# felixendres/rgbdslam_v2

Measured on AMD Instinct MI355X. Metric: frame-pairs matched+RANSAC/sec, 640x480 ORB-1000, higher is better.
Workload: dtype fp4 MFMA, exact (match) + f32/f64 (RANSAC); 1 GPU; configs[1]: synthetic 640x480 RGB-D, ORB 1000 kp, 20 candidate pairs/frame, 200 frames; max_matches=300, parallelism=pair-sharded x1, graph_capture=True

## Files before the change

rgbdslam_v2_amd/csrc/api_batches.hip:

```cpp
#include "rgbdfe_host.h"

namespace rgbdfe_host {


int fail(rgbdfe_ctx* ctx, int code, const std::string& msg) {
  if (ctx) {
    std::lock_guard<std::mutex> g(ctx->err_mu);
    ctx->last_error = msg;
  }
  return code;
}


void fill_ransac_const(rgbdfe_ctx* ctx) {
  const rgbdfe_params& p = ctx->cfg.params;
  RansacConst& rc = ctx->rc;
  rc.max_matches = p.max_matches;
  rc.min_matches = p.min_matches;
  rc.ransac_iterations = p.ransac_iterations;
  rc.max_dist_m = (float)(double)p.max_dist_for_inliers;
  rc.sq_max_dist = (double)(rc.max_dist_m * rc.max_dist_m);
  rc.depth_cov = p.depth_cov;
  const double cam_angle_x = 58.0 / 180.0 * M_PI;
  const double cam_angle_y = 45.0 / 180.0 * M_PI;
  const double cam_resol_x = 640;
  const double cam_resol_y = 480;
  const double sx = 3 * tan(cam_angle_x / cam_resol_x);
  const double sy = 3 * tan(cam_angle_y / cam_resol_y);
  rc.raster_cov_x = sx * sx;
  rc.raster_cov_y = sy * sy;
  rc.seed = p.seed;
  rc.g2o_iterations = (int32_t)p.g2o_iterations;
}

int validate_params(rgbdfe_ctx* ctx, const rgbdfe_params& p) {
  if (p.max_matches < 1 || p.max_matches > RGBDFE_MAX_MATCHES)
    return fail(ctx, RGBDFE_ERR_INVALID_ARG, "max_matches must be in [1, RGBDFE_MAX_MATCHES]");
  if (p.min_matches < 0 || p.ransac_iterations < 0)
    return fail(ctx, RGBDFE_ERR_INVALID_ARG, "min_matches / ransac_iterations must be >= 0");
  if (!(p.max_dist_for_inliers > 0.f))
    return fail(ctx, RGBDFE_ERR_INVALID_ARG, "max_dist_for_inliers must be > 0");
  if (p.g2o_iterations > 1000u) return fail(ctx, RGBDFE_ERR_INVALID_ARG, "g2o_iterations must be <= 1000");
  if (p.g2o_iterations > 0u && !(p.depth_cov > 0.0))
    return fail(ctx, RGBDFE_ERR_INVALID_ARG, "the g2o refinement needs depth_cov > 0");
  return RGBDFE_OK;
}

int ensure_scratch(rgbdfe_ctx* ctx, size_t bytes) {
  if (bytes <= ctx->scratch_bytes) return RGBDFE_OK;
  if (ctx->d_scratch) (void)hipFree(ctx->d_scratch);
  ctx->d_scratch = nullptr;
  ctx->scratch_bytes = 0;
  HIP_TRY(ctx, hipMalloc(&ctx->d_scratch, bytes));
  ctx->scratch_bytes = bytes;
  return RGBDFE_OK;
}

hipEvent_t get_event(rgbdfe_ctx* ctx) {
  if (!ctx->event_pool.empty()) {
    hipEvent_t e = ctx->event_pool.back();
    ctx->event_pool.pop_back();
    return e;
  }
  hipEvent_t e = nullptr;
  (void)hipEventCreate(&e);
  return e;
}

void drain_pending(rgbdfe_ctx* ctx) {
  for (auto& ln : ctx->lanes)
    if (ln.stream) (void)hipStreamSynchronize(ln.stream);
  for (auto& p : ctx->pending) {
    auto add = [&](int which, hipEvent_t e0, hipEvent_t e1) {
      float ms = 0.f;
      if (hipEventElapsedTime(&ms, e0, e1) == hipSuccess) {
        ctx->k_ms[which] += ms;
        ctx->k_launches[which]++;
        ctx->k_pairs[which] += p.pairs;
      }
    };
    if (p.sift) {
      add(RGBDFE_KERNEL_SIFT_DOT, p.a, p.b);
      add(RGBDFE_KERNEL_SIFT_FINISH, p.b, p.c);
      add(RGBDFE_KERNEL_RANSAC, p.c, p.d);
      ctx->event_pool.push_back(p.d);
    } else {
      add(RGBDFE_KERNEL_HAMMING, p.a, p.b);
      add(RGBDFE_KERNEL_RANSAC, p.b, p.c);
    }
    ctx->event_pool.push_back(p.a);
    ctx->event_pool.push_back(p.b);
    ctx->event_pool.push_back(p.c);
  }
  ctx->pending.clear();
}

int ensure_ec_pool(rgbdfe_ctx* ctx, rgbdfe_ctx::Lane& lane, size_t regions, hipStream_t stream) {
  if (regions <= lane.ec_regions) return RGBDFE_OK;
  HIP_TRY(ctx, hipStreamSynchronize(stream));
  if (lane.d_ec) (void)hipFree(lane.d_ec);
  lane.d_ec = nullptr;
  lane.ec_regions = 0;
  HIP_TRY(ctx, hipMalloc((void**)&lane.d_ec, regions * select_ransac_ec_region_bytes()));
  lane.ec_regions = regions;
  return RGBDFE_OK;
}
int want_latency_path(rgbdfe_ctx* ctx, rgbdfe_ctx::Lane& lane, int32_t n, hipStream_t stream, bool* use, int* chunk_out,
                      PhasePlan* plan) {
  const size_t need_recs = (size_t)n * (size_t)(ctx->rc.ransac_iterations > 0 ? ctx->rc.ransac_iterations : 0);
  const bool force_phases = ctx->latency_chunk_iters < 0;
  const int chunk_cfg = force_phases ? -ctx->latency_chunk_iters : ctx->latency_chunk_iters;
  int chunk = chunk_cfg > 0 ? chunk_cfg : (n <= 64 ? 4 : (n <= 640 ? 7 : (n <= 1280 ? 14 : 28)));
  const int I_all = ctx->rc.ransac_iterations > 0 ? ctx->rc.ransac_iterations : 0;
  const bool too_many_pairs = (size_t)n > kMaxEcRegions;
  while (!too_many_pairs && chunk < I_all && (size_t)n * (size_t)((I_all + chunk - 1) / chunk) > kMaxEcRegions) ++chunk;
  bool latency = !too_many_pairs && n <= ctx->latency_pairs && ctx->rc.ransac_iterations >= 2 * chunk &&
                 need_recs <= ((size_t)1 << 24);
  *chunk_out = chunk;
  if (latency && need_recs > lane.recs_capacity) {
    HIP_TRY(ctx, hipStreamSynchronize(stream));
    if (lane.d_recs) (void)hipFree(lane.d_recs);
    lane.d_recs = nullptr;
    lane.recs_capacity = 0;
    if (hipMalloc((void**)&lane.d_recs, need_recs * (sizeof(IterRec) + sizeof(IterSum)) +
                                            ransac_split_mask_bytes(need_recs, (size_t)ctx->cfg.max_pairs_per_batch)) == hipSuccess)
      lane.recs_capacity = need_recs;
    else latency = false;
  }
  if (latency && !lane.d_walk &&
      hipMalloc((void**)&lane.d_walk, sizeof(WalkState) * ((size_t)ctx->cfg.max_pairs_per_batch + 1)) != hipSuccess) {
    lane.d_walk = nullptr;
    latency = false;
  }
  const int I = ctx->rc.ransac_iterations;
  if (n <= 256 && !force_phases) { plan->n_phases = 1; plan->ends[0] = I; }
  else {
    const int cand[4] = {14, ((I * 7 / 20) / 7) * 7, ((I * 14 / 20) / 7) * 7, I};
    int k = 0, last = 0;
    for (int c : cand) { const int e = c > I ? I : c; if (e > last) { plan->ends[k++] = e; last = e; } }
    if (k == 0) plan->ends[k++] = I;
    plan->n_phases = k;
  }
  *use = latency;
  return ensure_ec_pool(ctx, lane, ((size_t)n + 7) / 8 * 8 + 8, stream);
}

bool hamming_on_mfma(const rgbdfe_ctx* ctx) { return ctx->hamming_mode != 0 && (uint32_t)ctx->cfg.max_keypoints <= 32768u; }

HammingGeometry hamming_geometry(const rgbdfe_ctx* ctx, uint32_t n, uint32_t max_nq, uint32_t max_nt) {
  const uint32_t cap = (uint32_t)ctx->cfg.max_pairs_per_batch;
  if (!hamming_on_mfma(ctx)) {
    HammingGeometry g = hamming_nn_geometry(n, max_nq, max_nt, cap);
    g.shape = 0;
    return g;
  }
  const int pipe_wide = ctx->hamming_mode == 4 ? 1 : ctx->hamming_mode == 3 ? ctx->hamming_wide : 0;
  return hamming_mfma_geometry(n, max_nq, max_nt, cap, pipe_wide, ctx->hamming_mode == 3 ? ctx->hamming_shape : 32);
}

uint32_t launch_hamming(rgbdfe_ctx* ctx, const PairWork* d_work, uint32_t* d_keys, uint32_t n, HammingGeometry geom,
                        hipStream_t stream) {
  const uint32_t mk = (uint32_t)ctx->cfg.max_keypoints;
  if (n > 0 && geom.qblocks > 0) { ctx->hamming_wide_last = (int)geom.wide; ctx->hamming_shape_last = (int)geom.shape; }
  if (hamming_on_mfma(ctx))
    return launch_hamming_mfma(ctx->d_desc4, d_work, d_keys, mk, n, geom, ctx->hamming_mode, stream);
  return launch_hamming_nn(ctx->d_desc, d_work, d_keys, mk, n, geom, stream);
}

uint32_t launch_hamming(rgbdfe_ctx* ctx, const PairWork* d_work, uint32_t* d_keys, uint32_t n, uint32_t max_nq,
                        uint32_t max_nt, hipStream_t stream) {
  return launch_hamming(ctx, d_work, d_keys, n, hamming_geometry(ctx, n, max_nq, max_nt), stream);
}

bool capture_stream_ready(rgbdfe_ctx* ctx) {
  if (ctx->capture_stream) return true;
  if (hipStreamCreateWithFlags(&ctx->capture_stream, hipStreamNonBlocking) != hipSuccess) { (void)hipGetLastError(); ctx->capture_stream = nullptr; }
  return ctx->capture_stream != nullptr;
}

int enqueue_pairs(rgbdfe_ctx* ctx, const int32_t* qids, const int32_t* tids, int32_t n, rgbdfe_match_result* d_out, hipEvent_t wait_for, int64_t* ticket_out, int* lane_out, int matcher, float* d_out_dist, double flann_ratio) {


  const bool sift = matcher != 0;
  if (n > ctx->cfg.max_pairs_per_batch)
    return fail(ctx, RGBDFE_ERR_CAPACITY, "n_pairs exceeds max_pairs_per_batch");
  const int64_t ticket = ctx->next_ticket;
  rgbdfe_ctx::Slot& slot = ctx->ring[ticket % rgbdfe_ctx::kRing];
  const int li = (int)(ticket % rgbdfe_ctx::kLanes);
  rgbdfe_ctx::Lane& lane = ctx->lanes[li];
  hipStream_t stream = lane.stream;
  if (slot.pending) {
    HIP_TRY(ctx, hipEventSynchronize(slot.done));
    slot.pending = false;
  }
  uint32_t max_nq = 0, max_nt = 0, sift_kinds = 0;
  for (int32_t i = 0; i < n; ++i) {
    auto q = ctx->nodes.find(qids[i]);
    auto t = ctx->nodes.find(tids[i]);
    if (q == ctx->nodes.end() || t == ctx->nodes.end())
      return fail(ctx, RGBDFE_ERR_UNKNOWN_NODE, "pair references a node that is not resident");
    if (q->second.kind != (uint32_t)matcher || t->second.kind != (uint32_t)matcher)
      return fail(ctx, RGBDFE_ERR_INVALID_ARG, "node descriptor kind does not fit this matcher");
    PairWork& w = slot.h_work[i];
    w.q_slot = q->second.slot;
    w.t_slot = t->second.slot;
    w.nq = q->second.n;
    w.nt = t->second.n;
    w.uid = pair_uid(qids[i], tids[i]);
    w.qid = qids[i];
    w.tid = tids[i];
    w.pad = matcher == 1 ? sift_fast_keys(ctx, q->second, t->second) : 0u;
    sift_kinds |= w.pad ? 1u : 2u;
    if (ctx->rc.g2o_iterations > 0 && !(q->second.flags & t->second.flags & kNodeHasKeypoints))
      return fail(ctx, RGBDFE_ERR_INVALID_ARG,
                  "g2o_iterations > 0: a node of the batch has no keypoints (rgbdfe_upload_node_keypoints after every upload of it)");
    if (w.nq > max_nq) max_nq = w.nq;
    if (w.nt > max_nt) max_nt = w.nt;
  }
  if (ctx->rc.g2o_iterations > 0 && !ctx->d_kp2d)
    return fail(ctx, RGBDFE_ERR_INVALID_ARG, "g2o_iterations > 0 needs the nodes' keypoints (rgbdfe_upload_node_keypoints)");
  int32_t piece = n;
  if (n > 0 && ctx->latency_pairs != 0) {
    const size_t I = (size_t)(ctx->rc.ransac_iterations > 0 ? ctx->rc.ransac_iterations : 1);
    size_t fit = (((size_t)1 << 24) / I) < kMaxEcRegions ? (((size_t)1 << 24) / I) : kMaxEcRegions;
    if (fit > 65535) fit = 65535;
    if (fit < 1) fit = 1;
    if ((size_t)n > fit && (size_t)n <= (size_t)ctx->latency_pairs) piece = (int32_t)fit;
  }
  if (sift && piece > 65535) return fail(ctx, RGBDFE_ERR_CAPACITY, "a one-wave SIFT batch holds at most 65535 pairs");
  bool latency = false;
  int chunk = 7;
  PhasePlan pp{};
  if (n > 0) {
    int rcl = want_latency_path(ctx, lane, piece, stream, &latency, &chunk, &pp);
    if (rcl != RGBDFE_OK) return rcl;
  }
  if (wait_for) HIP_TRY(ctx, hipStreamWaitEvent(stream, wait_for, 0));
  if (ctx->nodes_ready) HIP_TRY(ctx, hipStreamWaitEvent(stream, ctx->nodes_ready, 0));
  hipError_t launch_err = hipSuccess;
  if (n > 0) {
    if (!d_out) d_out = lane.d_results;
    const bool graphable = ctx->use_graphs && !sift && !ctx->profiling && piece >= n && ctx->rc.g2o_iterations == 0;
    const HammingGeometry geom = sift ? HammingGeometry{0, 1, 0}
                                      : hamming_geometry(ctx, (uint32_t)(piece < n ? piece : n), max_nq, max_nt);
    if (!sift && geom.qblocks > 0) { ctx->hamming_wide_last = (int)geom.wide; ctx->hamming_shape_last = (int)geom.shape; }
    rgbdfe_ctx::GraphEntry* ge = nullptr;
    bool capturing = false;
    if (graphable) {
      rgbdfe_ctx::GraphKey key;
      memset(&key, 0, sizeof(key));
      key.n = n; key.qblocks = geom.qblocks; key.tsplit = geom.tsplit; key.slot = (int32_t)(ticket % rgbdfe_ctx::kRing);
      key.latency = latency ? 1 : 0; key.chunk = chunk; key.hamming_mode = ctx->hamming_mode | (int32_t)(geom.wide << 8) | (int32_t)(geom.shape << 16); key.n_phases = pp.n_phases;
      for (int i = 0; i < 4; ++i) key.ends[i] = i < pp.n_phases ? pp.ends[i] : 0;
      memcpy(&key.rc, &ctx->rc, sizeof(RansacConst));
      key.d_out = d_out; key.d_recs = lane.d_recs; key.d_ec = lane.d_ec; key.d_walk = lane.d_walk; key.d_keys = lane.d_keys;
      size_t gi = 0;
      for (; gi < ctx->graphs.size(); ++gi)
        if (memcmp(&ctx->graphs[gi].key, &key, sizeof(key)) == 0) { ge = &ctx->graphs[gi]; break; }
      if (ge) {
        ge->used = ++ctx->graph_clock;
        const hipError_t le = hipGraphLaunch(ge->exec, stream);
        if (le == hipSuccess) {
          ctx->graph_launches++;
          ctx->graph_miss_run = 0;
        } else {
          (void)hipGetLastError();
          (void)hipGraphExecDestroy(ge->exec); (void)hipGraphDestroy(ge->graph);
          ctx->graphs.erase(ctx->graphs.begin() + (long)gi);
          ctx->graph_launch_failures++;
          ge = nullptr;
        }
      } else {
        ctx->graph_misses++;
        const bool try_capture = ctx->graph_miss_run < rgbdfe_ctx::kGraphMissRun ||
                                 ctx->graph_miss_run % rgbdfe_ctx::kGraphRetry == 0;
        ctx->graph_miss_run++;
        if (try_capture && capture_stream_ready(ctx) &&
            hipStreamBeginCapture(ctx->capture_stream, hipStreamCaptureModeRelaxed) == hipSuccess) {
          capturing = true;
          if (ctx->graphs.size() >= 48) {
            size_t lru = 0;
            for (size_t i = 1; i < ctx->graphs.size(); ++i) if (ctx->graphs[i].used < ctx->graphs[lru].used) lru = i;
            (void)hipGraphExecDestroy(ctx->graphs[lru].exec); (void)hipGraphDestroy(ctx->graphs[lru].graph);
            ctx->graphs.erase(ctx->graphs.begin() + (long)lru);
          }
          ctx->graphs.push_back(rgbdfe_ctx::GraphEntry{key, nullptr, nullptr, ++ctx->graph_clock});
        } else {
          (void)hipGetLastError();
          ctx->graph_plain_batches++;
        }
      }
    }
    rgbdfe_ctx::Pending pend{};
    pend.sift = sift;
    for (int attempt = 0; attempt < 2; ++attempt) {
      hipStream_t const ls = capturing ? ctx->capture_stream : stream;
      if (!ge) {
        const hipError_t me = hipMemcpyAsync(slot.d_work, slot.h_work, sizeof(PairWork) * (size_t)n, hipMemcpyHostToDevice, ls);
        if (me != hipSuccess && launch_err == hipSuccess) launch_err = me;
      }
      if (ctx->profiling) {
        pend.a = get_event(ctx);
        pend.b = get_event(ctx);
        pend.c = get_event(ctx);
        if (sift) pend.d = get_event(ctx);
        pend.pairs = n;
        (void)hipEventRecord(pend.a, ls);
      }
      const uint32_t mk = (uint32_t)ctx->cfg.max_keypoints;
      for (int32_t off = 0; off < n && !ge; off += piece) {
        const int32_t m = (n - off) < piece ? (n - off) : piece;
        const bool first = off == 0, last = off + m >= n;
        if (!first) {
          int rcl = want_latency_path(ctx, lane, m, ls, &latency, &chunk, &pp);
          if (rcl != RGBDFE_OK) { launch_err = hipErrorOutOfMemory; break; }
        }
        const PairWork* d_work = slot.d_work + off;
        rgbdfe_match_result* d_res = d_out + off;
        if (!sift) {
          const uint32_t planes = launch_hamming(ctx, d_work, lane.d_keys, (uint32_t)m, first ? geom : hamming_geometry(ctx, (uint32_t)m, max_nq, max_nt), ls);
          if (ctx->profiling && first) (void)hipEventRecord(pend.b, ls);
          if (latency)
            launch_select_ransac_latency(ctx->d_xyz, d_work, lane.d_keys, planes, d_res, mk, (uint32_t)m, ctx->rc,
                                         lane.d_prep, lane.d_recs, lane.d_walk, lane.d_ec, chunk, pp.ends, pp.n_phases, ls);
          else
            launch_select_ransac(ctx->d_xyz, d_work, lane.d_keys, planes, d_res, mk, (uint32_t)m, ctx->rc, lane.d_prep,
                                 lane.d_ec, ls);
          if (ctx->rc.g2o_iterations > 0)
            launch_g2o_refine(d_work, d_res, (uint32_t)m, ctx->rc, lane.d_prep, ctx->d_kp2d, mk, lane.d_ec, ls);
          if (ctx->profiling && last) (void)hipEventRecord(pend.c, ls);
        } else {
          float* d_dist = (d_out_dist ? d_out_dist : lane.d_all_dist) + (size_t)off * RGBDFE_MAX_MATCHES;
          if (matcher == 2) {
            launch_l2_knn2(ctx->d_sift_f32, d_work, mk, (uint32_t)m, max_nq, lane.d_row_part, ls);
            if (ctx->profiling && first) (void)hipEventRecord(pend.b, ls);
            launch_l2_ratio(d_work, mk, (uint32_t)m, lane.d_row_part, lane.d_col_part, flann_ratio, lane.d_sm_q,
                            lane.d_sm_t, lane.d_sm_d, lane.d_sm_n, ls);
          } else {
            launch_sift_dot(ctx->d_sift_bf16, d_work, mk, (uint32_t)m, max_nq, max_nt, sift_kinds, lane.d_row_part,
                            lane.d_col_part, lane.d_col_blocks, ls);
            if (ctx->profiling && first) (void)hipEventRecord(pend.b, ls);
            launch_sift_finish(ctx->d_sift_f32, d_work, mk, (uint32_t)m, lane.d_row_part, lane.d_col_part, lane.d_col_blocks,
                               lane.d_sm_q, lane.d_sm_t, lane.d_sm_d, lane.d_sm_n, ls);
          }
          if (ctx->profiling && first) (void)hipEventRecord(pend.c, ls);
          if (latency)
            launch_select_ransac_sift_latency(ctx->d_xyz, d_work, lane.d_sm_q, lane.d_sm_t, lane.d_sm_d, lane.d_sm_n,
                                              d_dist, d_res, mk, (uint32_t)m, ctx->rc,
                                              lane.d_prep, lane.d_recs, lane.d_walk, lane.d_ec, chunk, pp.ends, pp.n_phases, ls);
          else
            launch_select_ransac_sift(ctx->d_xyz, d_work, lane.d_sm_q, lane.d_sm_t, lane.d_sm_d,
                                      lane.d_sm_n, d_dist, d_res, mk,
                                      (uint32_t)m, ctx->rc, lane.d_prep, lane.d_ec, ls);
          if (ctx->rc.g2o_iterations > 0)
            launch_g2o_refine(d_work, d_res, (uint32_t)m, ctx->rc, lane.d_prep, ctx->d_kp2d, mk, lane.d_ec, ls);
          if (ctx->profiling && last) (void)hipEventRecord(pend.d, ls);
        }
      }
      if (capturing) {
        rgbdfe_ctx::GraphEntry& e = ctx->graphs.back();
        hipError_t ce = hipStreamEndCapture(ctx->capture_stream, &e.graph);
        if (ce == hipSuccess) ce = hipGraphInstantiate(&e.exec, e.graph, nullptr, nullptr, 0);
        if (ce == hipSuccess && launch_err == hipSuccess) {
          ctx->graph_captures++;
          ce = hipGraphLaunch(e.exec, stream);
          ctx->graph_launches++;
          if (ce != hipSuccess) launch_err = ce;
        } else {
          if (e.exec) (void)hipGraphExecDestroy(e.exec);
          if (e.graph) (void)hipGraphDestroy(e.graph);
          ctx->graphs.pop_back();
          (void)hipGetLastError();
          capturing = false;
          launch_err = hipSuccess;
          ctx->graph_capture_failures++;
          continue;
        }
      }
      break;
    }
    if (launch_err == hipSuccess) launch_err = hipGetLastError();
    if (ctx->profiling) {
      if (launch_err == hipSuccess) ctx->pending.push_back(pend);
      else {
        ctx->event_pool.push_back(pend.a); ctx->event_pool.push_back(pend.b); ctx->event_pool.push_back(pend.c);
        if (sift) ctx->event_pool.push_back(pend.d);
      }
    }
  }
  ctx->next_ticket++;
  slot.ticket = ticket;
  slot.failed = launch_err != hipSuccess;
  HIP_TRY(ctx, hipEventRecord(slot.done, stream));
  slot.pending = true;
  if (launch_err != hipSuccess)
    return fail(ctx, RGBDFE_ERR_HIP, std::string("kernel launch: ") + hipGetErrorString(launch_err));
  if (ticket_out) *ticket_out = ticket;
  if (lane_out) *lane_out = li;
  return RGBDFE_OK;
}

int wait_ticket(rgbdfe_ctx* ctx, int64_t ticket, hipStream_t stream) {
  if (ticket <= 0 || ticket >= ctx->next_ticket) return fail(ctx, RGBDFE_ERR_INVALID_ARG, "unknown ticket");
  rgbdfe_ctx::Slot& slot = ctx->ring[ticket % rgbdfe_ctx::kRing];
  if (slot.ticket == ticket && slot.failed) return fail(ctx, RGBDFE_ERR_HIP, "the batch with this ticket failed to launch");
  if (slot.ticket != ticket || !slot.pending) return RGBDFE_OK;
  if (stream) {
    HIP_TRY(ctx, hipStreamWaitEvent(stream, slot.done, 0));
  } else {
    HIP_TRY(ctx, hipEventSynchronize(slot.done));
    slot.pending = false;
  }
  return RGBDFE_OK;
}


}
```

rgbdslam_v2_amd/csrc/ransac_device.h:

```cpp
#pragma once
#include <float.h>
#include <stddef.h>

#include <type_traits>

#include "rgbdfe_internal.h"
#include "tfc_device.h"

namespace rgbdfe {

constexpr int kWave = 64;
constexpr int kRounds = RGBDFE_MAX_MATCHES / kWave;

constexpr int kSlots = 7;
constexpr int kFitUnroll = 4;
constexpr int kOrdStride = RGBDFE_MAX_MATCHES + 2 * kFitUnroll + 4;
static_assert(kOrdStride % 4 == 0 && (kOrdStride / 4) % 2 == 1, "list rows: word aligned, odd word count");
static_assert(RGBDFE_MAX_MATCHES <= 512, "list entries keep the low 8 bits of a match index + one threshold");

struct FitBuf {
  uint8_t ord[kSlots][kOrdStride];
};

__device__ __forceinline__ uint32_t mix32(uint32_t x) {
// ... 136 lines not shown
  return ((uint64_t)hi << 32) | lo;
}

__device__ __forceinline__ int fit_compact(int s, const uint64_t* mask, const uint64_t* w_nonzero, FitBuf& fit,
                                           int& n_below_256, int lane) {
  uint32_t base = 0;
  n_below_256 = 0;
#pragma unroll
  for (int r = 0; r < kRounds; ++r) {
    const uint64_t pm = mask[r] & w_nonzero[r];
    if (__builtin_amdgcn_inverse_ballot_w64(pm)) fit.ord[s][base + lane_rank(pm)] = (uint8_t)(r * kWave + lane);
    base += (uint32_t)__popcll(pm);
    if (r == 256 / kWave - 1) n_below_256 = (int)base;
  }
  if (lane < 2 * kFitUnroll) fit.ord[s][base + lane] = 0;
  return (int)base;
}

__device__ __forceinline__ void pin(float& v) { asm volatile("" : "+v"(v)); }

template <bool FAST_DIV>
__device__ __forceinline__ void fit_recurrence(int n_mine, int k256_mine, int n_min, int n_max, const FitBuf& fit,
                                               const float* __restrict__ M, float& C, float& m1, float& m2, int lane) {
  constexpr int U = kFitUnroll;
  const int sl = min(lane / 9, kSlots - 1);
  const int l9 = lane % 9;
  const int ci = l9 / 3, cj = l9 % 3;
  const uint8_t* __restrict__ ord = fit.ord[sl];
  auto rec_off = [&](int k) {
    const uint32_t hi = (k >= k256_mine) ? 256u * kRecBytes : 0u;
    return (uint32_t)ord[k] * kRecBytes + hi;
  };
  const char* __restrict__ recs = reinterpret_cast<const char*>(M);
  const char* __restrict__ recP = recs + cj * 4;
  const char* __restrict__ recQ = recs + 12 + ci * 4;
  float W = 0.0f;
  C = 0.0f; m1 = 0.0f; m2 = 0.0f;
  uint32_t off[U];
  float wv[U], fv[U], tv[U];
#pragma unroll
  for (int u = 0; u < U; ++u) off[u] = rec_off(u);
#pragma unroll
  for (int u = 0; u < U; ++u) {
    wv[u] = *reinterpret_cast<const float*>(recs + off[u] + 24);
    fv[u] = *reinterpret_cast<const float*>(recP + off[u]);
    tv[u] = *reinterpret_cast<const float*>(recQ + off[u]);
  }
#pragma unroll
  for (int u = 0; u < U; ++u) off[u] = rec_off(U + u);
  auto trip = [&](int k0, auto with_select) {
    float wc[U], fc[U], tc[U];
#pragma unroll
    for (int u = 0; u < U; ++u) { wc[u] = wv[u]; fc[u] = fv[u]; tc[u] = tv[u]; }
#pragma unroll
    for (int u = 0; u < U; ++u) {
      wv[u] = *reinterpret_cast<const float*>(recs + off[u] + 24);
      fv[u] = *reinterpret_cast<const float*>(recP + off[u]);
      tv[u] = *reinterpret_cast<const float*>(recQ + off[u]);
    }
#pragma unroll
    for (int u = 0; u < U; ++u) off[u] = rec_off(k0 + 2 * U + u);
    float al[U], om[U];
#pragma unroll
    for (int u = 0; u < U; ++u) {
      W = W + wc[u];
      if (FAST_DIV) {
        float r = __builtin_amdgcn_rcpf(W);
        const float e = __builtin_fmaf(-W, r, 1.0f);
        r = __builtin_fmaf(e, r, r);
        float q = wc[u] * r;
        float res = __builtin_fmaf(-W, q, wc[u]);
        q = __builtin_fmaf(res, r, q);
        res = __builtin_fmaf(-W, q, wc[u]);
        al[u] = __builtin_fmaf(res, r, q);
      } else {
        al[u] = wc[u] / W;
      }
      om[u] = 1.0f - al[u];
    }
#pragma unroll
    for (int u = 0; u < U; ++u) {
      const bool act = (k0 + u) < n_mine;
      const float d1 = fc[u] - m1;
      const float d2 = tc[u] - m2;
      const float outer = d2 * d1;
      const float scaled = al[u] * outer;
      const float sum = C + scaled;
      float Cn = om[u] * sum;
      float m1n = m1 + al[u] * d1;
      float m2n = m2 + al[u] * d2;
      if (decltype(with_select)::value) {
        pin(Cn); pin(m1n); pin(m2n);
        C = act ? Cn : C;
        m1 = act ? m1n : m1;
        m2 = act ? m2n : m2;
      } else {
        C = Cn; m1 = m1n; m2 = m2n;
      }
    }
  };
  int k0 = 0;
  for (; k0 + U <= n_min; k0 += U) trip(k0, std::false_type());
  for (; k0 < n_max; k0 += U) trip(k0, std::true_type());
}

__device__ __forceinline__ uint32_t prescreen_may_pass(const float* hypR, const float* hypt, const float* __restrict__ M,
                                                    int n_all, float pmax, const RansacConst& rc) {
  const float u4 = 4.0f * 5.9604645e-8f;
  float es = 0.0f;
#pragma unroll
  for (int i = 0; i < 3; ++i)
    es += u4 * (((fabsf(hypR[3 * i]) + fabsf(hypR[3 * i + 1])) + fabsf(hypR[3 * i + 2]) + 1.0f) * pmax + fabsf(hypt[i]));
  const double smax = rc.raster_cov_x > rc.depth_cov ? rc.raster_cov_x : rc.depth_cov;
  const float S = (float)(2.0 * (smax + smax));
  const float E = 2.0f * ((2.0f * sqrtf(S) * 1.001f) * es + es * es + u4 * S) + 1e-30f;
  const float hi_f = S * 1.000001f + E;
  uint32_t may_pass = 0;
  typedef float v2f __attribute__((ext_vector_type(2)));
  v2f R2[9], t2[3];
#pragma unroll
  for (int i = 0; i < 9; ++i) R2[i] = v2f{hypR[i], hypR[i]};
#pragma unroll
  for (int i = 0; i < 3; ++i) t2[i] = v2f{hypt[i], hypt[i]};
#pragma unroll 1
  for (int m0 = 0; m0 < n_all; m0 += 4) {
    float rec[4][6];
#pragma unroll
    for (int u = 0; u < 4; ++u)
#pragma unroll
      for (int c = 0; c < 6; ++c) rec[u][c] = M[(m0 + u) * kRec + c];
#pragma unroll
    for (int u = 0; u < 4; u += 2) {
      const v2f px = {rec[u][0], rec[u + 1][0]}, py = {rec[u][1], rec[u + 1][1]}, pz = {rec[u][2], rec[u + 1][2]};
      const v2f qx = {rec[u][3], rec[u + 1][3]}, qy = {rec[u][4], rec[u + 1][4]}, qz = {rec[u][5], rec[u + 1][5]};
      const v2f f0 = __builtin_elementwise_fma(R2[0], px, __builtin_elementwise_fma(R2[1], py, __builtin_elementwise_fma(R2[2], pz, t2[0]))) - qx;
      const v2f f1 = __builtin_elementwise_fma(R2[3], px, __builtin_elementwise_fma(R2[4], py, __builtin_elementwise_fma(R2[5], pz, t2[1]))) - qy;
      const v2f f2 = __builtin_elementwise_fma(R2[6], px, __builtin_elementwise_fma(R2[7], py, __builtin_elementwise_fma(R2[8], pz, t2[2]))) - qz;
      const v2f dsq = __builtin_elementwise_fma(f0, f0, __builtin_elementwise_fma(f1, f1, f2 * f2));
      may_pass += !(dsq.x > hi_f) ? 1u : 0u;
      may_pass += !(dsq.y > hi_f) ? 1u : 0u;
    }
  }
  return may_pass;
}

constexpr int kS4Block = 24;
__device__ __forceinline__ void transpose_records(const float* __restrict__ M, float* __restrict__ S4, int tid, int n_threads) {
  for (int v = tid; v < (RGBDFE_MAX_MATCHES / 4) * kS4Block; v += n_threads) {
    const int blk = v / kS4Block, r = v - blk * kS4Block;
    S4[v] = M[(blk * 4 + (r & 3)) * kRec + (r >> 2)];
  }
}
__device__ __forceinline__ uint32_t prescreen_may_pass_s4(const float* hypR, const float* hypt, const float* __restrict__ S4,
                                                       int n_all, float pmax, const RansacConst& rc) {
  const float u4 = 4.0f * 5.9604645e-8f;
  float es = 0.0f;
#pragma unroll
  for (int i = 0; i < 3; ++i)
    es += u4 * (((fabsf(hypR[3 * i]) + fabsf(hypR[3 * i + 1])) + fabsf(hypR[3 * i + 2]) + 1.0f) * pmax + fabsf(hypt[i]));
  const double smax = rc.raster_cov_x > rc.depth_cov ? rc.raster_cov_x : rc.depth_cov;
  const float S = (float)(2.0 * (smax + smax));
  const float E = 2.0f * ((2.0f * sqrtf(S) * 1.001f) * es + es * es + u4 * S) + 1e-30f;
  const float hi_f = S * 1.000001f + E;
  uint32_t may_pass = 0;
  typedef float v2f __attribute__((ext_vector_type(2)));
  typedef float v4f __attribute__((ext_vector_type(4)));
  v2f R2[9], t2[3];
#pragma unroll
  for (int i = 0; i < 9; ++i) R2[i] = v2f{hypR[i], hypR[i]};
#pragma unroll
  for (int i = 0; i < 3; ++i) t2[i] = v2f{hypt[i], hypt[i]};
  const v4f* __restrict__ blocks = reinterpret_cast<const v4f*>(S4);
#pragma unroll 1
  for (int m0 = 0; m0 < n_all; m0 += 4) {
    const v4f* __restrict__ b = blocks + (m0 >> 2) * 6;
    const v4f px = b[0], py = b[1], pz = b[2], qx = b[3], qy = b[4], qz = b[5];
#pragma unroll
    for (int h = 0; h < 2; ++h) {
      const v2f x = h ? px.zw : px.xy, y = h ? py.zw : py.xy, z = h ? pz.zw : pz.xy;
      const v2f f0 = __builtin_elementwise_fma(R2[0], x, __builtin_elementwise_fma(R2[1], y, __builtin_elementwise_fma(R2[2], z, t2[0]))) - (h ? qx.zw : qx.xy);
      const v2f f1 = __builtin_elementwise_fma(R2[3], x, __builtin_elementwise_fma(R2[4], y, __builtin_elementwise_fma(R2[5], z, t2[1]))) - (h ? qy.zw : qy.xy);
      const v2f f2 = __builtin_elementwise_fma(R2[6], x, __builtin_elementwise_fma(R2[7], y, __builtin_elementwise_fma(R2[8], z, t2[2]))) - (h ? qz.zw : qz.xy);
      const v2f dsq = __builtin_elementwise_fma(f0, f0, __builtin_elementwise_fma(f1, f1, f2 * f2));
      may_pass += !(dsq.x > hi_f) ? 1u : 0u;
      may_pass += !(dsq.y > hi_f) ? 1u : 0u;
    }
  }
  return may_pass;
}

struct WalkRegs {
  int it, real_iterations, valid_iterations, best_idx, best_n;
  float rmse;
  bool done;
};
template <bool COHERENT, class Listed>
__device__ __forceinline__ void walk_records(WalkRegs& w, int recorded_end, int I, int n_all, uint32_t thr,
                                             const IterSum* __restrict__ sum_pair, Listed listed, int lane) {
  while (!w.done && w.it < I && w.real_iterations < recorded_end) {
    const int k0 = w.real_iterations;
    const int G = min(kWave, recorded_end - k0);
    int rn_l = 0;
    double rerr_l = 0.0;
    if (lane < G && listed(k0 + lane)) {
      if (COHERENT) {
        const unsigned long long* p = reinterpret_cast<const unsigned long long*>(sum_pair + (k0 + lane));
        const unsigned long long a = __hip_atomic_load(p, __ATOMIC_RELAXED, __HIP_MEMORY_SCOPE_AGENT);
        const unsigned long long b = __hip_atomic_load(p + 1, __ATOMIC_RELAXED, __HIP_MEMORY_SCOPE_AGENT);
        rerr_l = __longlong_as_double((long long)a);
        rn_l = (int)(uint32_t)b;
      } else {
        const IterSum su = sum_pair[k0 + lane];
        rn_l = su.rn;
        rerr_l = su.rerr;
      }
    }
    const uint64_t with_matches = __ballot(lane < G && rn_l > 0);
    for (int g = 0; g < G;) {
      const uint64_t rest = with_matches >> g;
      const int run = rest != 0ull ? (int)__builtin_ctzll(rest) : G - g;
      if (run > 0) {
        const int can = min(run, max(I - w.it, 0));
        w.real_iterations += can;
        w.it += can;
        if (can < run) { w.done = true; break; }
        g += run;
        if (g >= G) break;
      }
      if (!(w.it < I)) { w.done = true; break; }
      w.real_iterations++;
      const int refined_n = __builtin_amdgcn_readlane(rn_l, g);
      const double refined_error = __hiloint2double(__builtin_amdgcn_readlane(__double2hiint(rerr_l), g),
                                                    __builtin_amdgcn_readlane(__double2loint(rerr_l), g));
      w.valid_iterations++;
      if (refined_error <= (double)w.rmse && refined_n >= w.best_n && (uint32_t)refined_n >= thr) {
        w.rmse = (float)refined_error;
        w.best_idx = k0 + g;
        w.best_n = refined_n;
        if ((double)refined_n > (double)n_all * 0.5) w.it += 10;
        if ((double)refined_n > (double)n_all * 0.75) w.it += 10;
        if ((double)refined_n > (double)n_all * 0.8) { w.done = true; break; }
      }
      ++w.it;
      ++g;
    }
  }
}

#ifndef RGBDFE_CLASS2_NUM
#define RGBDFE_CLASS2_NUM 9
#define RGBDFE_CLASS2_DEN 14
#endif
constexpr int kClass2Num = RGBDFE_CLASS2_NUM, kClass2Den = RGBDFE_CLASS2_DEN;

}
```

rgbdslam_v2_amd/csrc/ransac_split.hip:

```cpp
#include <stdio.h>
#include <stdlib.h>

#include <mutex>
#include <vector>

#include "ransac_device.h"

namespace rgbdfe {

namespace {

__device__ __forceinline__ void lsync() {
  __builtin_amdgcn_wave_barrier();
  asm volatile("s_waitcnt lgkmcnt(0)" ::: "memory");
  __builtin_amdgcn_wave_barrier();
}

__device__ __forceinline__ void lds_barrier() {
  asm volatile("s_waitcnt lgkmcnt(0)\n\ts_barrier" ::: "memory");
}

__device__ __forceinline__ int fresh(int v) {
  asm volatile("" : "+v"(v));
  return v;
}

constexpr int kHypThreads = 256;

#ifdef RGBDFE_SPLIT_STATS
__device__ unsigned long long g_split_stats[40];
#define ST_DECL unsigned long long st_c[40] = {0, 0, 0, 0, 0, 0, 0, 0, 0, 0, 0, 0, 0, 0, 0, 0, 0, 0, 0, 0, 0, 0, 0, 0, 0, 0, 0, 0, 0, 0, 0, 0, 0, 0, 0, 0, 0, 0, 0, 0}, st_mx = 0;
#define ST_ADD(I, V) { st_c[I] += (unsigned long long)(V); }
#define ST_MAX(I, V) { st_mx = (unsigned long long)(V) > st_mx ? (unsigned long long)(V) : st_mx; }
#define ST_T0 unsigned long long st_t = __builtin_amdgcn_s_memrealtime();
#define ST_LAP(I) { const unsigned long long st_n = __builtin_amdgcn_s_memrealtime(); st_c[I] += st_n - st_t; st_t = st_n; }
#define ST_OUT { if ((threadIdx.x & 63) == 0) { for (int st_i = 0; st_i < 40; ++st_i) if (st_c[st_i] != 0ull) atomicAdd(&g_split_stats[st_i], st_c[st_i]); \
                 if (st_mx != 0ull) atomicMax(&g_split_stats[7], st_mx); } }
#else
#define ST_DECL
#define ST_ADD(I, V)
#define ST_MAX(I, V)
#define ST_T0
#define ST_LAP(I)
#define ST_OUT
#endif

#ifndef RGBDFE_SPLIT_WAVES
#define RGBDFE_SPLIT_WAVES 8
#endif
constexpr int kStreamWaves = RGBDFE_SPLIT_WAVES;
#ifndef RGBDFE_SPLIT_WGS_PER_CU
#define RGBDFE_SPLIT_WGS_PER_CU (16 / RGBDFE_SPLIT_WAVES)
#endif
constexpr int kWgsPerCu = RGBDFE_SPLIT_WGS_PER_CU;
static_assert(kStreamWaves >= 3 && (kStreamWaves * kWgsPerCu) % 4 == 0, "whole waves per SIMD");
#define RGBDFE_SPLIT_EU_WAVES (RGBDFE_SPLIT_WAVES * RGBDFE_SPLIT_WGS_PER_CU / 4)
constexpr int kWorkers = kStreamWaves - 1;
#ifndef RGBDFE_SPLIT_SERVER_SCORES
#define RGBDFE_SPLIT_SERVER_SCORES (RGBDFE_SPLIT_WAVES >= 8)
#endif
constexpr bool kServerScores = RGBDFE_SPLIT_SERVER_SCORES;
constexpr int kStreamThreads = kStreamWaves * kWave;
#ifndef RGBDFE_SPLIT_WAVE_SLOTS
#define RGBDFE_SPLIT_WAVE_SLOTS 7
#endif
#ifndef RGBDFE_SPLIT_BUFS
#define RGBDFE_SPLIT_BUFS (RGBDFE_SPLIT_WAVES >= 8 ? 4 : 2)
#endif
constexpr int kWaveSlots = RGBDFE_SPLIT_WAVE_SLOTS;
static_assert(kWaveSlots <= kSlots, "the refit phase (fit_compact / fit_recurrence) holds kSlots lists per wave");
constexpr int kGroupSlots = kWorkers * kWaveSlots;
constexpr int kStreamSlots = 2 * kGroupSlots;
static_assert(kGroupSlots <= kWave, "the server looks at a group's slots with one lane each");
static_assert(kStreamSlots <= 2 * kWave, "the server's end-of-work test looks at two slots per lane");
#ifndef RGBDFE_SPLIT_TICKETS_FROM
#define RGBDFE_SPLIT_TICKETS_FROM (24 * (RGBDFE_SPLIT_WAVES - 1) * RGBDFE_SPLIT_WAVE_SLOTS / 49)
#endif
constexpr int kCostDear = 4;
constexpr int kTicketsFrom = RGBDFE_SPLIT_TICKETS_FROM;
#ifndef RGBDFE_SPLIT_PACK_FROM
#define RGBDFE_SPLIT_PACK_FROM 1000
#endif
constexpr int kPackFrom = RGBDFE_SPLIT_PACK_FROM;
constexpr int kBufs = RGBDFE_SPLIT_BUFS;
#ifndef RGBDFE_SPLIT_MAX_SHARE
#define RGBDFE_SPLIT_MAX_SHARE 256
#endif
constexpr int kMaxShare = RGBDFE_SPLIT_MAX_SHARE;
constexpr int kMaskLanes = kMaxShare / kWave + 1;
constexpr int kMVec = RGBDFE_MAX_MATCHES * kRec / 4;
constexpr int kPrepVec = (int)(sizeof(PairPrep) / 16);
static_assert(sizeof(PairPrep) % 16 == 0, "PairPrep goes global -> LDS in 16-byte pieces");

constexpr int kSlotDone = 0, kSlotActive = 1, kSlotRecorded = 2;
struct SlotS {
  union {
    struct { float R[9], t[3]; } x;
    float svd_in[15];
  } u;
  uint64_t cmask[kRounds];
  double rerr;
  double csum;
  int rn;
  int cn;
  int active;
  int round;
  int iter;
  int buf;
  uint32_t pair;
  int n_all;
  uint32_t thr;
  float pmax;
};
struct ScoreB {
  uint16_t cand[RGBDFE_MAX_MATCHES];
  uint32_t mbits[2 * kRounds];
  uint32_t pad[2];
  double err[RGBDFE_MAX_MATCHES + 8];
};
static_assert(offsetof(ScoreB, err) % 16 == 0, "16-byte reads of the error list");
struct alignas(16) WaveLds {
  union {
    ScoreB sc;
    FitBuf fit;
  } u;
};
constexpr int kUnitFree = 0, kUnitLoading = 1, kUnitReady = 2, kUnitDrained = 3;
struct alignas(16) UnitCtx {
  uint64_t mw[kMaskLanes + 1];
  int state;
  int next;
  int done;
  int n_items;
  uint32_t pair;
  int kb, ke;
  uint32_t thr;
  int base;
  int cls;
  int w_it, w_real, w_valid, w_best_idx, w_best_n, w_state;
  float w_rmse;
  int pad[3];
  uint16_t klist[kMaxShare];
};
struct alignas(16) StreamLds {
  PairPrep prep[kBufs];
  WaveLds w[kServerScores ? kStreamWaves : kWorkers];
  SlotS slot[kStreamSlots];
  UnitCtx ctx[kBufs];
  int claim_nall[kWave];
  int claim_cls[kWave];
  uint8_t act_list[2][kWave];
  int n_act[2];
  int task[2];
  int tickets[2];
  uint8_t wlist[2][kWorkers][8];
  int quit[2];
  int sum_rn[2];
  uint16_t ord_cnt[kWave], ord_start[kWave];
#ifdef RGBDFE_SPLIT_STATS
  unsigned int st_w[2][8][2];
#endif
};
static_assert(sizeof(StreamLds) <= 160 * 1024 / kWgsPerCu, "kWgsPerCu workgroups per CU");

__device__ __forceinline__ void score_b(const float* R, const float* tr, const float* __restrict__ M, int n_all,
                                        uint32_t need, const RansacConst& rc, ScoreB& sb, float pmax, uint64_t* mask,
                                        int& n_inl, double& sum, int& n_cand_out) {
  const int lane = threadIdx.x & (kWave - 1);
  double Rd[9], td[3];
#pragma unroll
  for (int i = 0; i < 9; ++i) Rd[i] = (double)R[i];
#pragma unroll
  for (int i = 0; i < 3; ++i) td[i] = (double)tr[i];
  const double rcx = rc.raster_cov_x, rcy = rc.raster_cov_y, dc = rc.depth_cov;
  const double smax = rcx > dc ? rcx : dc;
  const double shortcut = 2.0 * (smax + smax);
  float lo_f, hi_f;
  {
    const float u4 = 4.0f * 5.9604645e-8f;
    float es = 0.0f;
#pragma unroll
    for (int i = 0; i < 3; ++i)
      es += u4 * (((fabsf(R[3 * i]) + fabsf(R[3 * i + 1])) + fabsf(R[3 * i + 2]) + 1.0f) * pmax + fabsf(tr[i]));
    const float S = (float)shortcut;
    const float E = 2.0f * ((2.0f * sqrtf(S) * 1.001f) * es + es * es + u4 * S) + 1e-30f;
    lo_f = S * 0.999999f - E;
    hi_f = S * 1.000001f + E;
  }
  int n_cand = 0;
  float rec[kRounds][6];
#pragma unroll
  for (int r = 0; r < kRounds; ++r) {
    const int m = r * kWave + lane;
#pragma unroll
    for (int c = 0; c < 6; ++c) rec[r][c] = M[m * kRec + c];
  }
  bool pre[kRounds], cand[kRounds];
  bool unsure = false;
#pragma unroll
  for (int r = 0; r < kRounds; ++r) {
    const int m = r * kWave + lane;
    const float pxf = rec[r][0], pyf = rec[r][1], pzf = rec[r][2];
    const float qxf = rec[r][3], qyf = rec[r][4], qzf = rec[r][5];
    pre[r] = (m < n_all) && !(pzf == 0.0f || qzf == 0.0f) && !(__builtin_isnan(pzf) || __builtin_isnan(qzf));
    const float f0 = __builtin_fmaf(R[0], pxf, __builtin_fmaf(R[1], pyf, __builtin_fmaf(R[2], pzf, tr[0]))) - qxf;
    const float f1 = __builtin_fmaf(R[3], pxf, __builtin_fmaf(R[4], pyf, __builtin_fmaf(R[5], pzf, tr[1]))) - qyf;
    const float f2 = __builtin_fmaf(R[6], pxf, __builtin_fmaf(R[7], pyf, __builtin_fmaf(R[8], pzf, tr[2]))) - qzf;
    const float dsq_f = __builtin_fmaf(f0, f0, __builtin_fmaf(f1, f1, f2 * f2));
    const bool sure_in = dsq_f < lo_f, sure_out = dsq_f > hi_f;
    cand[r] = pre[r] && sure_in;
    unsure = unsure || (pre[r] && !(sure_in || sure_out));
  }
  if (__ballot(unsure) != 0ull) {
#pragma unroll
    for (int r = 0; r < kRounds; ++r) {
      const float pxf = rec[r][0], pyf = rec[r][1], pzf = rec[r][2];
      const float qxf = rec[r][3], qyf = rec[r][4], qzf = rec[r][5];
      const double a0 = (double)pxf, a1 = (double)pyf, a2 = (double)pzf;
      const double d0 = (((Rd[0] * a0 + Rd[1] * a1) + Rd[2] * a2) + td[0]) - (double)qxf;
      const double d1 = (((Rd[3] * a0 + Rd[4] * a1) + Rd[5] * a2) + td[1]) - (double)qyf;
      const double d2 = (((Rd[6] * a0 + Rd[7] * a1) + Rd[8] * a2) + td[2]) - (double)qzf;
      const double dsq = (d0 * d0 + d1 * d1) + d2 * d2;
      cand[r] = pre[r] && !(dsq > shortcut) && !__builtin_isnan(d2);
    }
  }
#pragma unroll
  for (int r = 0; r < kRounds; ++r) {
    const uint64_t cm = __ballot(cand[r]);
    if (cand[r]) sb.cand[n_cand + (int)lane_rank(cm)] = (uint16_t)(r * kWave + lane);
    n_cand += __popcll(cm);
  }
  if (lane < 2 * kRounds) sb.mbits[lane] = 0u;
  lsync();
  n_inl = 0;
  sum = 0.0;
#pragma unroll
  for (int r = 0; r < kRounds; ++r) mask[r] = 0ull;
  n_cand_out = n_cand;
  if ((uint32_t)n_cand < need) return;
  for (int k0 = 0; k0 < n_cand; k0 += kWave) {
    const int k = k0 + lane;
    const bool act = k < n_cand;
    const int m = act ? (int)sb.cand[k] : 0;
    const double a0 = (double)M[m * kRec + 0], a1 = (double)M[m * kRec + 1], a2 = (double)M[m * kRec + 2];
    const double b0 = (double)M[m * kRec + 3], b1 = (double)M[m * kRec + 4], b2 = (double)M[m * kRec + 5];
    double d[3];
    d[0] = (((Rd[0] * a0 + Rd[1] * a1) + Rd[2] * a2) + td[0]) - b0;
    d[1] = (((Rd[3] * a0 + Rd[4] * a1) + Rd[5] * a2) + td[1]) - b1;
    d[2] = (((Rd[6] * a0 + Rd[7] * a1) + Rd[8] * a2) + td[2]) - b2;
    double e = DBL_MAX;
    {
      const double c1[3] = {rcx * a2, rcy * a2, dc};
      const double c2[3] = {rcx * b2, rcy * b2, dc};
      double A[9];
#pragma unroll
      for (int i = 0; i < 3; ++i)
#pragma unroll
        for (int kk = 0; kk < 3; ++kk) A[i * 3 + kk] = Rd[kk * 3 + i] * c1[kk];
      const double S00 = ((A[0] * Rd[0] + A[1] * Rd[3]) + A[2] * Rd[6]) + c2[0];
      const double S10 = (A[3] * Rd[0] + A[4] * Rd[3]) + A[5] * Rd[6];
      const double S11 = ((A[3] * Rd[1] + A[4] * Rd[4]) + A[5] * Rd[7]) + c2[1];
      const double S20 = (A[6] * Rd[0] + A[7] * Rd[3]) + A[8] * Rd[6];
      const double S21 = (A[6] * Rd[1] + A[7] * Rd[4]) + A[8] * Rd[7];
      const double S22 = ((A[6] * Rd[2] + A[7] * Rd[5]) + A[8] * Rd[8]) + c2[2];
      bool ok, unsafe;
      double ee = mahal_llt_fast(S00, S10, S11, S20, S21, S22, d, ok, unsafe);
      if (__ballot(act && unsafe) != 0ull)
        ee = mahal_llt_ieee(S00, S10, S11, S20, S21, S22, d, ok);
      if (ok && (ee >= 0.0)) e = ee;
    }
    const bool inl = act && !(e > rc.sq_max_dist) && (e >= 0.0);
    const uint64_t im = __ballot(inl);
    if (inl) {
      sb.err[n_inl + (int)lane_rank(im)] = e;
      atomicOr(&sb.mbits[m >> 5], 1u << (m & 31));
    }
    n_inl += __popcll(im);
  }
  if (lane < 8) sb.err[n_inl + lane] = 0.0;
  lsync();
#pragma unroll
  for (int r = 0; r < kRounds; ++r) {
    const uint32_t lo = __builtin_amdgcn_readfirstlane(sb.mbits[2 * r]);
    const uint32_t hi = __builtin_amdgcn_readfirstlane(sb.mbits[2 * r + 1]);
    mask[r] = ((uint64_t)hi << 32) | lo;
  }
  if (!((uint32_t)n_inl < need || n_inl < 3)) {
    double s = 0.0;
    for (int k = 0; k < n_inl; k += 8) {
      const double2 v0 = *reinterpret_cast<const double2*>(&sb.err[k]);
      const double2 v1 = *reinterpret_cast<const double2*>(&sb.err[k + 2]);
      const double2 v2 = *reinterpret_cast<const double2*>(&sb.err[k + 4]);
      const double2 v3 = *reinterpret_cast<const double2*>(&sb.err[k + 6]);
      s += v0.x; s += v0.y; s += v1.x; s += v1.y;
      s += v2.x; s += v2.y; s += v3.x; s += v3.y;
    }
    sum = s;
  }
  lsync();
}

}

__global__ __launch_bounds__(kHypThreads) void ransac_hyp_kernel(const PairWork* __restrict__ work, uint32_t n_pairs,
                                                                const RansacConst rc, const SplitPlan plan) {
  __shared__ __attribute__((aligned(16))) float M[RGBDFE_MAX_MATCHES * kRec];
  __shared__ __attribute__((aligned(16))) float S4[(RGBDFE_MAX_MATCHES / 4) * kS4Block];
  const uint32_t pair = blockIdx.x;
  if (pair >= n_pairs) return;
  if (pair == 0 && threadIdx.x < sizeof(WalkState) / 4) reinterpret_cast<uint32_t*>(plan.walk + n_pairs)[threadIdx.x] = 0u;
  const PairPrep* __restrict__ pp = plan.prep + pair;
  const int n_all = pp->n_all;
  if (threadIdx.x == 0) {
    WalkState ws;
    ws.state = rc.ransac_iterations;
    ws.it = 0; ws.real_iterations = 0; ws.valid_iterations = 0;
    ws.best_idx = -1; ws.best_n = 0;
    ws.rmse = 1e6f;
    ws.speculate = plan.phased ? 0 : rc.ransac_iterations;
    plan.walk[pair] = ws;
  }
  if (!(n_all > rc.min_matches && n_all >= 4)) return;
  const int tid = threadIdx.x, lane = tid & (kWave - 1);
  {
    const float4* __restrict__ src = reinterpret_cast<const float4*>(pp->M);
    float4* __restrict__ dst = reinterpret_cast<float4*>(M);
    for (int v = tid; v < kMVec; v += kHypThreads) dst[v] = src[v];
  }
  __shared__ int n_viable_sh;
  if (tid == 0) n_viable_sh = 0;
  __syncthreads();
  transpose_records(M, S4, tid, kHypThreads);
  __syncthreads();
  const float pmax = pp->pmax;
  uint32_t thr = (uint32_t)rc.min_matches;
  if ((double)thr > 0.75 * (double)n_all) thr = (uint32_t)(0.75 * (double)n_all);
  const uint32_t seed_uid = mix32(mix32(rc.seed ^ 0x9E3779B9u) + work[pair].uid * 0x85EBCA6Bu);
  const int I = rc.ransac_iterations;
  IterRec* __restrict__ rec_pair = plan.recs + (size_t)pair * (size_t)I;
  uint64_t* __restrict__ vm_pair = plan.vmask + (size_t)pair * (size_t)plan.vmask_words;
  int n_viable_wave = 0;
  for (int k0 = 0; k0 < I; k0 += kHypThreads) {
    const int k = k0 + tid;
    const bool in_range = k < I;
    const uint32_t iter = (uint32_t)k;
    uint32_t ids[4] = {0, 0, 0, 0};
    int cnt = 0;
    {
      int safety_net = 0;
      uint32_t kk = 0;
      const uint32_t n = (uint32_t)n_all;
      while (cnt < 4) {
        uint32_t id1 = rand31(seed_uid, iter, kk) % n;
        uint32_t id2 = rand31(seed_uid, iter, kk + 1) % n;
        kk += 2;
        if (id1 > id2) id1 = id2;
        const bool dup = (cnt > 0 && ids[0] == id1) || (cnt > 1 && ids[1] == id1) || (cnt > 2 && ids[2] == id1);
        if (!dup) {
          uint32_t v = id1;
#pragma unroll
          for (int s4 = 0; s4 < 4; ++s4) {
            if (s4 < cnt) {
              if (ids[s4] > v) { uint32_t tmp = ids[s4]; ids[s4] = v; v = tmp; }
            } else if (s4 == cnt) {
              ids[s4] = v;
            }
          }
          ++cnt;
        }
        if (++safety_net > 10000) break;
      }
    }
    Tfc acc;
    acc.reset();
#pragma unroll
    for (int s4 = 0; s4 < 4; ++s4)
      if (s4 < cnt) acc.add(M, (int)ids[s4]);
    float hypR[9], hypt[3];
    tfc_get_transformation(acc, hypR, hypt);
    const uint32_t may_pass = prescreen_may_pass_s4(hypR, hypt, S4, n_all, pmax, rc);
    const bool viable = in_range && !has_nan12(hypR, hypt) && may_pass >= thr;
    const uint64_t vm = __ballot(viable);
    if (lane == 0) vm_pair[k >> 6] = vm;
    n_viable_wave += __popcll(vm);
    if (k0 == 0 && tid < kWave && plan.preclass_iters > 0) {
      const int n14 = min(plan.preclass_iters, min(I, kWave));
      uint32_t best = (lane < n14 && viable) ? may_pass : 0u;
#pragma unroll
      for (int d = 32; d >= 1; d >>= 1) best = max(best, (uint32_t)__shfl_xor((int)best, d));
      const int viable14 = __popcll(vm & (n14 >= 64 ? ~0ull : ((1ull << n14) - 1ull)));
      if (lane == 0)
        plan.preclass[pair] = (viable14 * kClass2Den <= n14 * kClass2Num && best * 10u <= (uint32_t)n_all * 3u) ? 2 : 0;
    }
    if (viable) {
      IterRec& r = rec_pair[k];
#pragma unroll
      for (int i = 0; i < 9; ++i) r.rR[i] = hypR[i];
#pragma unroll
      for (int i = 0; i < 3; ++i) r.rt[i] = hypt[i];
#ifdef RGBDFE_PROFILE_PHASES
      r.rn = -77;
#endif
    }
  }
  if (plan.phased) {
    if (lane == 0) atomicAdd(&n_viable_sh, n_viable_wave);
    __syncthreads();
    if (tid == 0) {
      const int b = order_bucket(n_viable_sh);
      const uint32_t at = atomicAdd(plan.order_cnt + b, 1u);
      if (at < n_pairs) plan.order[(size_t)b * (size_t)n_pairs + at] = pair;
    }
  }
}

__global__ __launch_bounds__(kStreamThreads) __attribute__((amdgpu_waves_per_eu(RGBDFE_SPLIT_EU_WAVES, RGBDFE_SPLIT_EU_WAVES))) void ransac_refine_kernel(
    uint32_t n_pairs, const RansacConst rc, const SplitPlan plan, uint32_t n_units) {
  extern __shared__ __attribute__((aligned(16))) char stream_smem[];
  StreamLds& lds = *reinterpret_cast<StreamLds*>(stream_smem);
  const int lane = threadIdx.x & (kWave - 1);
  const int wave = __builtin_amdgcn_readfirstlane((int)(threadIdx.x >> 6));
  const int I = rc.ransac_iterations;
  ST_DECL

  if (wave < 2) {
    const int s = wave * kWave + lane;
    if (s < kStreamSlots) { lds.slot[s].active = kSlotDone; lds.slot[s].iter = -1; lds.slot[s].buf = 0; }
    if (wave == 0 && lane < kBufs) { lds.ctx[lane].state = kUnitFree; lds.ctx[lane].next = 0; lds.ctx[lane].done = 0; lds.ctx[lane].n_items = 0; }
    if (wave == 0 && lane < 2) lds.quit[lane] = 0;
  }
  lds_barrier();

  auto write_summary = [&](const SlotS& sl) {
    plan.sums[(size_t)sl.pair * (size_t)I + (size_t)sl.iter] = IterSum{sl.rerr, sl.rn, 0};
  };
  auto accept_record = [&](const SlotS& sl, int n_inl, double err) {
    IterRec& r = plan.recs[(size_t)sl.pair * (size_t)I + (size_t)sl.iter];
#pragma unroll
    for (int i = 0; i < 9; ++i) r.rR[i] = sl.u.x.R[i];
#pragma unroll
    for (int i = 0; i < 3; ++i) r.rt[i] = sl.u.x.t[i];
#pragma unroll
    for (int q = 0; q < kRounds; ++q) r.rmask[q] = sl.cmask[q];
    r.rerr = err;
    r.rn = n_inl;
    r.pad = 0;
  };

  auto score_slot = [&](SlotS& sl) {
    WaveLds& wl = lds.w[wave];
    float curR[9], curt[3];
#pragma unroll
    for (int i = 0; i < 9; ++i) curR[i] = sl.u.x.R[i];
#pragma unroll
    for (int i = 0; i < 3; ++i) curt[i] = sl.u.x.t[i];
    const int b = __builtin_amdgcn_readfirstlane(sl.buf);
    const PairPrep& pp = lds.prep[b];
    const int n_all = __builtin_amdgcn_readfirstlane(sl.n_all);
    const uint32_t thr = (uint32_t)__builtin_amdgcn_readfirstlane((int)sl.thr);
    const float pmax = __int_as_float(__builtin_amdgcn_readfirstlane(__float_as_int(sl.pmax)));
    const uint32_t need = max(thr, (uint32_t)__builtin_amdgcn_readfirstlane(sl.rn));
    uint64_t inl_mask[kRounds];
    int n_inl;
    double sum;
    int n_cand;
    score_b(curR, curt, pp.M, n_all, need, rc, wl.u.sc, pmax, inl_mask, n_inl, sum, n_cand);
#ifdef RGBDFE_SPLIT_STATS
    ST_ADD(29, n_cand)
    if ((uint32_t)n_cand >= need) {
      ST_ADD(26, 1) ST_ADD(27, (n_cand + 63) / 64)
      if (!((uint32_t)n_inl < need || n_inl < 3)) ST_ADD(28, n_inl)
    }
#endif
    if (fresh(threadIdx.x & (kWave - 1)) == 0) {
#pragma unroll
      for (int r = 0; r < kRounds; ++r) sl.cmask[r] = inl_mask[r];
      sl.cn = n_inl;
      sl.csum = sum;
    }
  };
  auto score_tickets = [&](int g) {
    const int n_act = __builtin_amdgcn_readfirstlane(lds.n_act[g]);
    for (;;) {
      int t = 0;
      if (fresh(threadIdx.x & (kWave - 1)) == 0) t = atomicAdd(&lds.task[g], 1);
      t = __builtin_amdgcn_readfirstlane(t);
      if (t >= n_act) break;
      score_slot(lds.slot[g * kGroupSlots + (int)lds.act_list[g][t]]);
    }
  };

  if (wave < kWorkers) {
    WaveLds& wl = lds.w[wave];
    lds_barrier();
    ST_T0
    for (int h = 0;; ++h) {
      const int g = h & 1;
      const int lane = fresh(threadIdx.x & (kWave - 1));
#ifdef RGBDFE_SPLIT_STATS
      const unsigned long long st_s0 = st_c[16], st_f0 = st_c[17];
#endif
      const int n_mine_slots = __builtin_amdgcn_readfirstlane((int)lds.wlist[g][wave][7]);
      const int my_slot = g * kGroupSlots + (lane < n_mine_slots ? (int)lds.wlist[g][wave][min(lane, kWaveSlots - 1)] : 0);
      auto slot_at = [&](int j) -> SlotS& { return lds.slot[__builtin_amdgcn_readlane(my_slot, j)]; };
      if (__builtin_amdgcn_readfirstlane(lds.tickets[g]) != 0) {
        score_tickets(g);
        ST_LAP(16)
        lds_barrier();
        ST_LAP(18)
      } else {
        for (int j = 0; j < n_mine_slots; ++j) score_slot(slot_at(j));
        lsync();
        ST_LAP(16)
      }
      bool still = false;
      if (fresh(lane) < n_mine_slots) {
        SlotS& sl = lds.slot[my_slot];
        if (sl.active == kSlotActive) {
          const int n_inl = sl.cn, rn = sl.rn;
          const uint32_t thr = sl.thr;
          const uint32_t need = max(thr, (uint32_t)rn);
          const double err_mine = !((uint32_t)n_inl < need || n_inl < 3) ? sqrt(sl.csum / (double)n_inl) : 1e9;
          float max_dist_f = rc.max_dist_m;
          asm volatile("" : "+v"(max_dist_f));
          if (!((uint32_t)n_inl < thr || err_mine > (double)max_dist_f)) {
            if (n_inl >= rn && err_mine <= sl.rerr) {
              still = (n_inl != rn);
              accept_record(sl, n_inl, err_mine);
              sl.rn = n_inl;
              sl.rerr = err_mine;
            }
          }
          if (sl.round == 18) still = false;
// ... 406 lines not shown
#pragma unroll
      for (int e = 0; e < 6; ++e) v[e] = hyp[e];
#pragma unroll
      for (int e = 0; e < 6; ++e) reinterpret_cast<float2*>(sl.u.x.R)[e] = v[e];
      uint32_t rerr_hi = 0x412E8480u;
      asm volatile("" : "+v"(rerr_hi));
      reinterpret_cast<uint32_t*>(&sl.rerr)[0] = 0u;
      reinterpret_cast<uint32_t*>(&sl.rerr)[1] = rerr_hi;
      sl.rn = 0;
      sl.active = kSlotActive;
      sl.round = 0;
      sl.iter = k;
      sl.buf = b;
      sl.pair = cx.pair;
      sl.n_all = lds.prep[b].n_all;
      sl.thr = cx.thr;
      sl.pmax = lds.prep[b].pmax;
    }
    lsync();
  };

  auto sum_refined = [&](int gs) {
    const int lane = fresh(threadIdx.x & (kWave - 1));
    const SlotS& sl = lds.slot[gs * kGroupSlots + min(lane, kGroupSlots - 1)];
    int v = (lane < kGroupSlots && sl.iter >= 0 && sl.active == kSlotActive) ? sl.rn : 0;
#pragma unroll
    for (int d = 32; d >= 1; d >>= 1) v += __shfl_xor(v, d);
    if (lane == 0) lds.sum_rn[gs] = v;
    lsync();
  };

  auto deal_work = [&](int gs) {
    const int lane = fresh(threadIdx.x & (kWave - 1));
    const SlotS& sl = lds.slot[gs * kGroupSlots + min(lane, kGroupSlots - 1)];
    const bool a = lane < kGroupSlots && sl.iter >= 0 && sl.active == kSlotActive;
    const bool dear = a && sl.rn > 0;
    const uint64_t m = __ballot(a), dm = __ballot(dear), cm = m & ~dm;
    if (a) lds.act_list[gs][lane_rank(m)] = (uint8_t)lane;
    const int D = __popcll(dm), Cn = __popcll(cm);
    const bool packed = kPackFrom >= 0 && D >= 4 && __builtin_amdgcn_readfirstlane(lds.sum_rn[gs]) >= kPackFrom;
    if (lane == 0) {
      lds.n_act[gs] = D + Cn;
      lds.task[gs] = 0;
      lds.tickets[gs] = (packed || D >= kTicketsFrom) ? 1 : 0;
    }
    const int q = D / kWorkers, r = D - q * kWorkers;
    const int L = r > 0 ? kWorkers - r : 0;
    const int fill = kCostDear * L;
    int w = 0, pos = 0;
    if (dear) {
      const int d = (int)lane_rank(dm);
      w = d % kWorkers;
      pos = d / kWorkers;
    } else if (a) {
      const int c = (int)lane_rank(cm);
      if (c < fill) {
        w = r + c % L;
        pos = q + c / L;
      } else {
        const int c2 = c - fill, n1 = min(fill, Cn);
        w = c2 % kWorkers;
        const int first = (w >= r && L > 0) ? (n1 / L + ((w - r) < n1 % L ? 1 : 0)) : 0;
        pos = (w < r ? q + 1 : q) + first + c2 / kWorkers;
      }
    }
    if (packed) {
      const int idx = dear ? (int)lane_rank(dm) : D + (int)lane_rank(cm);
      w = idx / kWaveSlots;
      pos = idx - w * kWaveSlots;
    }
    if (__ballot(a && pos >= kWaveSlots) != 0ull) {
      const int p = (int)lane_rank(m);
      w = p % kWorkers;
      pos = p / kWorkers;
    }
    if (a) lds.wlist[gs][w][pos] = (uint8_t)lane;
    int cnt = 0;
#pragma unroll
    for (int k = 0; k < kWorkers; ++k) {
      const int ck = __popcll(__ballot(a && w == k));
      if (lane == k) cnt = ck;
    }
    if (lane < kWorkers) lds.wlist[gs][lane][7] = (uint8_t)cnt;
  };

  if (lane < 2) { lds.n_act[lane] = 0; lds.task[lane] = 0; lds.tickets[lane] = 0; }
  prefetch_block();
  adopt_block();
  issue_loads();
  complete_loads();
  advance_units();
  hand_out(0);
  sum_refined(0);
  deal_work(0);
  issue_loads();
  lds_barrier();
  ST_T0
  for (int h = 0;; ++h) {
    const int g = h & 1, gs = 1 - g;
    const int by_ticket = __builtin_amdgcn_readfirstlane(lds.tickets[g]);
    ST_ADD(0, 1) ST_ADD(2, by_ticket) ST_ADD(3, lds.n_act[g])
    ST_LAP(15)
    serve_svd(gs);
    ST_LAP(8)
#ifndef RGBDFE_SPLIT_NO_EARLY_MID
    if (by_ticket) {
      if (kServerScores) score_tickets(g);
      ST_LAP(14)
      lds_barrier();
    }
#endif
    recycle(gs);
    ST_LAP(9)
    complete_loads();
    advance_units();
    ST_LAP(10)
    hand_out(gs);
    ST_LAP(11)
    sum_refined(gs);
    deal_work(gs);
    ST_LAP(12)
    issue_loads();
    ST_LAP(13)
    const int lane = fresh(threadIdx.x & (kWave - 1));
    bool busy = lane < kBufs && lds.ctx[min(lane, kBufs - 1)].state != kUnitFree;
    busy = busy || (lane < kStreamSlots && lds.slot[min(lane, kStreamSlots - 1)].iter >= 0) ||
           (lane + kWave < kStreamSlots && lds.slot[min(lane + kWave, kStreamSlots - 1)].iter >= 0);
    const bool more = __ballot(busy) != 0ull || live != 0ull || nx_n != 0 || units_left;
    if (!more && lane == 0) lds.quit[g] = 1;
#ifdef RGBDFE_SPLIT_NO_EARLY_MID
    if (by_ticket) {
      if (kServerScores) score_tickets(g);
      ST_LAP(14)
      lds_barrier();
    }
#endif
    lds_barrier();
    ST_LAP(15)
#ifdef RGBDFE_SPLIT_STATS
    {
      unsigned int ms = 0, mf = 0, mb = 0, ss = 0, sf = 0;
      for (int wk = 0; wk < kWorkers; ++wk) {
        const unsigned int a = lds.st_w[g][wk][0], b = lds.st_w[g][wk][1];
        ms = a > ms ? a : ms; mf = b > mf ? b : mf; mb = a + b > mb ? a + b : mb; ss += a; sf += b;
      }
      ST_ADD(30, ms) ST_ADD(31, ss / kWorkers) ST_ADD(32, mf) ST_ADD(33, sf / kWorkers) ST_ADD(34, mb) ST_ADD(35, (ss + sf) / kWorkers)
    }
#endif
    if (!more) { ST_ADD(1, 1) ST_MAX(7, h + 1) ST_OUT break; }
  }
}

void launch_ransac_hyp(const PairWork* work, uint32_t n_pairs, const RansacConst& rc, const SplitPlan& plan,
                       hipStream_t stream) {
  if (n_pairs == 0) return;
  hipLaunchKernelGGL(ransac_hyp_kernel, dim3(n_pairs), dim3(kHypThreads), 0, stream, work, n_pairs, rc, plan);
}

int ransac_split_init() {
  static int n_cus[64] = {};
  static std::mutex mu;
  int dev = 0;
  if (hipGetDevice(&dev) != hipSuccess || dev < 0 || dev >= 64) dev = 0;
  std::lock_guard<std::mutex> g(mu);
  if (n_cus[dev] == 0) {
    int v = 0;
    if (hipDeviceGetAttribute(&v, hipDeviceAttributeMultiprocessorCount, dev) != hipSuccess || v <= 0) v = 256;
#ifdef RGBDFE_SPLIT_ONE_WG_PER_CU
    (void)hipFuncSetAttribute(reinterpret_cast<const void*>(ransac_refine_kernel), hipFuncAttributeMaxDynamicSharedMemorySize, 100 * 1024);
#else
    (void)hipFuncSetAttribute(reinterpret_cast<const void*>(ransac_refine_kernel), hipFuncAttributeMaxDynamicSharedMemorySize,
                              (int)sizeof(StreamLds));
#endif
    if (getenv("RGBDFE_SPLIT_VERBOSE")) {
      int nb = -1;
      const hipError_t e = hipOccupancyMaxActiveBlocksPerMultiprocessor(&nb, reinterpret_cast<const void*>(ransac_refine_kernel), kStreamThreads, sizeof(StreamLds));
      fprintf(stderr, "ransac_refine_kernel: %zu B LDS per workgroup, %d workgroups per CU (%s), %d CUs (device %d)\n", sizeof(StreamLds), nb, hipGetErrorString(e), v, dev);
    }
    n_cus[dev] = v;
  }
  return n_cus[dev];
}

void launch_ransac_refine(uint32_t n_pairs, const RansacConst& rc, const SplitPlan& plan_in, hipStream_t stream) {
  SplitPlan plan = plan_in;
  if (!plan.phased && plan.share_iters > kMaxShare) {
    const int I = rc.ransac_iterations > 0 ? rc.ransac_iterations : 0;
    plan.n_shares = I > 0 ? (I + kMaxShare - 1) / kMaxShare : 1;
    plan.share_iters = I > 0 ? (I + plan.n_shares - 1) / plan.n_shares : kMaxShare;
  }
  const uint32_t units = n_pairs * (uint32_t)plan.n_shares;
  if (units == 0) return;
  const uint32_t max_wgs = (uint32_t)ransac_split_wgs();
#ifdef RGBDFE_SPLIT_ONE_WG_PER_CU
  const size_t lds_bytes = 100 * 1024;
#else
  const size_t lds_bytes = sizeof(StreamLds);
#endif
  hipLaunchKernelGGL(ransac_refine_kernel, dim3(units < max_wgs ? units : max_wgs), dim3(kStreamThreads), lds_bytes, stream,
                     n_pairs, rc, plan, units);
}

int ransac_split_words_per_pair(int ransac_iterations) {
  const int I = ransac_iterations > 0 ? ransac_iterations : 0;
  return 4 * ((I + kHypThreads - 1) / kHypThreads);
}
int ransac_split_max_share() { return kMaxShare; }
int ransac_split_wgs() { return kWgsPerCu * ransac_split_init(); }

}

#ifdef RGBDFE_SPLIT_STATS
extern "C" int rgbdfe_debug_split_stats(unsigned long long* out40, int reset) {
  if (out40 && hipMemcpyFromSymbol(out40, HIP_SYMBOL(rgbdfe::g_split_stats), 320) != hipSuccess) return -1;
  if (reset) {
    unsigned long long z[40] = {};
    if (hipMemcpyToSymbol(HIP_SYMBOL(rgbdfe::g_split_stats), z, 320) != hipSuccess) return -1;
  }
  return 0;
}
#endif
```

rgbdslam_v2_amd/csrc/rgbdfe_host.h:

```cpp
#pragma once
#include <hip/hip_runtime.h>

#include <algorithm>
#include <atomic>
#include <climits>
#include <cmath>
#include <cstdint>
#include <cstdio>
#include <cstdlib>
#include <cstring>
#include <condition_variable>
#include <functional>
#include <memory>
#include <mutex>
#include <thread>
#include <string>
#include <unordered_map>
#include <unordered_set>
#include <vector>

#include "fast_host.h"
#include "orb_host.h"
#include "sift_extract.h"
#include "rgbdfe_internal.h"
#include "sensor_host.h"

using namespace rgbdfe;

namespace rgbdfe_host {

struct CloudEntry {
  float4* d = nullptr;
  int ch = 0, cw = 0;
  float fx = 0, fy = 0, cx = 0, cy = 0;
  int cloud_skip = 1;
  float4* d_samples = nullptr;
  int samples_skip = 0;
};

inline double erf_boundary(double target) {
  double lo = -8.0, hi = 8.0;
  for (;;) {
    const double mid = lo + (hi - lo) * 0.5;
    if (!(mid > lo && mid < hi)) break;
    if (0.5 * (1 + std::erf(mid)) >= target) hi = mid; else lo = mid;
  }
  return hi;
}

inline double division_boundary(double q, double denom) {
  double c = q * denom;
  while (c / denom >= q) c = std::nextafter(c, -INFINITY);
  while (c / denom < q) c = std::nextafter(c, INFINITY);
  return c;
}

struct NodeEntry {
  uint32_t slot;
  uint32_t n;
  uint32_t kind;
  uint32_t flags = 0;
};
constexpr uint32_t kNodeHasKeypoints = 2u;

inline uint32_t mix32_host(uint32_t x) {
  x ^= x >> 16; x *= 0x7feb352du;
  x ^= x >> 15; x *= 0x846ca68bu;
  x ^= x >> 16;
  return x;
}
inline uint32_t pair_uid(int32_t qid, int32_t tid) {
  return mix32_host((uint32_t)qid * 0x9E3779B1u ^ ((uint32_t)tid + 0x7F4A7C15u));
}

}
using namespace rgbdfe_host;

namespace rgbdfe_host {

class TaskPool {
 public:
  explicit TaskPool(int n) {
    for (int i = 0; i < n; ++i) th_.emplace_back([this] { run(); });
  }
  ~TaskPool() {
    { std::lock_guard<std::mutex> l(m_); stop_ = true; }
    cv_.notify_all();
    for (auto& t : th_) if (t.joinable()) t.join();
  }
  void submit(std::function<void()> f) {
    { std::lock_guard<std::mutex> l(m_); q_.push_back(std::move(f)); ++pending_; }
    cv_.notify_one();
  }
  void wait_all() {
    std::unique_lock<std::mutex> l(m_);
    done_.wait(l, [&] { return pending_ == 0; });
  }
  int size() const { return (int)th_.size(); }
 private:
  void run() {
    for (;;) {
      std::function<void()> f;
      {
        std::unique_lock<std::mutex> l(m_);
        cv_.wait(l, [&] { return stop_ || !q_.empty(); });
        if (stop_ && q_.empty()) return;
        f = std::move(q_.front());
        q_.erase(q_.begin());
      }
      try { f(); } catch (...) { failed_ = true; }
      { std::lock_guard<std::mutex> l(m_); --pending_; }
      done_.notify_all();
    }
  }
  std::vector<std::thread> th_;
  std::vector<std::function<void()>> q_;
  std::mutex m_;
  std::condition_variable cv_, done_;
  int pending_ = 0;
  bool stop_ = false;
 public:
  bool failed_ = false;
};

}
using namespace rgbdfe_host;

inline hipError_t create_side_stream(hipStream_t* s, int which) {
  int lo = 0, hi = 0;
  if (hipDeviceGetStreamPriorityRange(&lo, &hi) != hipSuccess || lo == hi) { (void)hipGetLastError(); return hipStreamCreateWithFlags(s, hipStreamNonBlocking); }
  return hipStreamCreateWithPriority(s, hipStreamNonBlocking, which > 0 ? hi : lo);
}

struct rgbdfe_ctx {
  rgbdfe_config cfg{};
  std::mutex mu;
  std::mutex err_mu;
  std::string last_error;
  struct Group* group = nullptr;
  hipStream_t stream = nullptr;
  uint32_t* d_desc = nullptr;
  float4* d_xyz = nullptr;
  uint32_t* d_desc4 = nullptr;
  float* d_kp2d = nullptr;
  hipStream_t orb_upload_stream = nullptr;
  hipStream_t orb_compute_stream = nullptr;
  hipEvent_t orb_upload_done[OrbWorkspace::kSets] = {};
  hipEvent_t orb_describe_done[OrbWorkspace::kSets] = {};
  bool feature_min_depth = false;
  bool sift_fast = true;
  int hamming_mode = RGBDFE_HAMMING_MODE_DEFAULT;
  int hamming_wide = -1;
  int hamming_wide_last = -1;
  int hamming_shape = 0;
  int hamming_shape_last = -1;
#ifndef RGBDFE_LANES
#define RGBDFE_LANES 2
#endif
  static constexpr int kLanes = RGBDFE_LANES;
  static constexpr int kRing = 2 * RGBDFE_LANES;
  struct Lane {
    hipStream_t stream = nullptr;
    IterRec* d_recs = nullptr;
    size_t recs_capacity = 0;
    WalkState* d_walk = nullptr;
    PairPrep* d_prep = nullptr;
    double* d_ec = nullptr;
    size_t ec_regions = 0;
    uint32_t* d_keys = nullptr;
    rgbdfe_match_result* d_results = nullptr;
    uint32_t* d_row_part = nullptr;
    uint32_t* d_col_part = nullptr;
    uint2* d_col_blocks = nullptr;
    uint16_t* d_sm_q = nullptr;
    uint16_t* d_sm_t = nullptr;
    float* d_sm_d = nullptr;
    int32_t* d_sm_n = nullptr;
    float* d_all_dist = nullptr;
  };
  uint16_t* d_sift_bf16 = nullptr;
  float* d_sift_f32 = nullptr;
  bool sift_ready = false;
  struct Slot {
    PairWork* h_work = nullptr;
    PairWork* d_work = nullptr;
    hipEvent_t done = nullptr;
    bool pending = false;
    bool failed = false;
    int64_t ticket = 0;
  };
  Lane lanes[kLanes];
  Slot ring[kRing];
  int32_t latency_pairs = INT32_MAX;
  int32_t latency_chunk_iters = 0;
  int64_t next_ticket = 1;
  struct GraphKey {
    int32_t n; uint32_t qblocks, tsplit; int32_t slot, latency, chunk, hamming_mode, n_phases; int32_t ends[4];
    RansacConst rc;
    void* d_out; void* d_recs; void* d_ec; void* d_walk; void* d_keys;
  };
  struct GraphEntry { GraphKey key; hipGraph_t graph; hipGraphExec_t exec; uint64_t used; };
  std::vector<GraphEntry> graphs;
  uint64_t graph_clock = 0;
  int64_t graph_launches = 0, graph_captures = 0;
  int64_t graph_misses = 0;
  int64_t graph_plain_batches = 0;
  int64_t graph_launch_failures = 0;
  int32_t graph_miss_run = 0;
  static constexpr int32_t kGraphMissRun = 8, kGraphRetry = 16;
  bool use_graphs = false;
  hipStream_t capture_stream = nullptr;
  long graph_capture_failures = 0;
  uint8_t* upload_stage = nullptr; size_t upload_stage_bytes = 0;
  hipEvent_t ev_in = nullptr;
  hipEvent_t nodes_ready = nullptr;
  hipEvent_t nodes_ready_ev = nullptr;
  rgbdfe_match_result* h_results = nullptr;
  struct HostJob {
    bool pending = false;
    bool waiting = false;
    bool direct = false;
    int payload = 0;
    int64_t ticket = 0;
    int32_t n = 0;
    void* out = nullptr;
    size_t out_bytes = 0;
    hipEvent_t copied = nullptr;
  };
  HostJob host_jobs[kLanes];
  uint8_t* h_stage[kLanes] = {};
  uint8_t* d_inl_stream[kLanes] = {};
  int32_t* d_inl_total[kLanes] = {};
  int32_t* h_inl_total[kLanes] = {};
  void* d_scratch = nullptr;
  size_t scratch_bytes = 0;
  void* d_icp = nullptr;
  size_t icp_bytes = 0;
  OrbWorkspace orb;
  OrbWorkspace orb_super;
  std::unique_ptr<TaskPool> detect_pool, stage_pool;
  SiftExtractor sift2, sift3;
  hipStream_t sift_stream1 = nullptr, sift_stream2 = nullptr, sift_stream3 = nullptr;
  SiftExtractor sift;
  struct SiftNodeBufs {
    size_t plane = 0;
    float* h_depth = nullptr; float* d_depth = nullptr;
    int32_t* d_n = nullptr; int32_t* h_n = nullptr;
    float4* d_xyz_out = nullptr; float* d_feat_out = nullptr; int32_t* d_kept_out = nullptr;
    float4* h_xyz_out = nullptr; float* h_feat_out = nullptr; int32_t* h_kept_out = nullptr;
    hipStream_t depth_stream = nullptr;
    hipEvent_t depth_done[3] = {};
  } sn;
  struct SiftBehindBufs {
    size_t plane = 0; int rows_per_frame = 0, agg_per_frame = 0;
    void* dev = nullptr; void* pin = nullptr;
    float* d_qdesc = nullptr; float4* d_qkeys = nullptr; size_t q_cap = 0;
  } sb;
  struct SiftOrbBufs {
    int rows = 0, cols = 0;
    void* dev = nullptr; void* pin = nullptr;
    int8_t* d_pattern = nullptr;
  } so;
  struct SensorBufs {
    static constexpr int kPinned = 6, kDevice = 3;
    uint8_t* h_raw[kPinned] = {}; size_t h_cap[kPinned] = {};
    uint8_t* d_raw[kDevice] = {}; size_t d_cap[kDevice] = {};
    float* d_depth[2] = {}; size_t depth_cap[2] = {};
    uint8_t* d_planes = nullptr; size_t planes_cap = 0;
    int32_t* d_maps = nullptr; size_t maps_cap = 0;
    int maps_key[4] = {0, 0, 0, 0};
  } sensor;
  int orb_max_keypoints = 0;
  int32_t detector_type = RGBDFE_DETECTOR_ORB;
  FastWorkspace fast;
  std::unordered_map<int32_t, NodeEntry> nodes;
  std::unordered_map<int32_t, CloudEntry> clouds;
  double emm_q_lo = 0.0, emm_q_hi = 0.0;
  std::vector<uint32_t> free_slots;
  RansacConst rc{};
  bool profiling = false;
  hipEvent_t ev[3] = {nullptr, nullptr, nullptr};
  double k_ms[RGBDFE_KERNEL_COUNT] = {};
  int64_t k_launches[RGBDFE_KERNEL_COUNT] = {};
  int64_t k_pairs[RGBDFE_KERNEL_COUNT] = {};
  struct Pending { hipEvent_t a, b, c, d; int32_t pairs; bool sift; };
  std::vector<Pending> pending;
  std::vector<hipEvent_t> event_pool;
};

namespace rgbdfe_host {
inline TaskPool& stage_pool(rgbdfe_ctx* ctx) {
  static const int n = getenv("RGBDFE_STAGE_THREADS") ? std::max(1, atoi(getenv("RGBDFE_STAGE_THREADS"))) : 4;
  if (!ctx->stage_pool) ctx->stage_pool.reset(new TaskPool(n));
  return *ctx->stage_pool;
}
inline uint32_t sift_fast_keys(const rgbdfe_ctx* ctx, const NodeEntry& q, const NodeEntry& t) {
  return (ctx->sift_fast && (q.flags & t.flags & 1u) && q.n <= 1024u && t.n <= 1024u) ? 1u : 0u;
}
}


using namespace rgbdfe_host;

namespace rgbdfe_host {
struct PhasePlan { int ends[4]; int n_phases; };
constexpr size_t kMaxEcRegions = (size_t)1 << 16;
int fail(rgbdfe_ctx* ctx, int code, const std::string& msg);
void fill_ransac_const(rgbdfe_ctx* ctx);
int validate_params(rgbdfe_ctx* ctx, const rgbdfe_params& p);
int ensure_scratch(rgbdfe_ctx* ctx, size_t bytes);
hipEvent_t get_event(rgbdfe_ctx* ctx);
void drain_pending(rgbdfe_ctx* ctx);
int ensure_ec_pool(rgbdfe_ctx* ctx, rgbdfe_ctx::Lane& lane, size_t regions, hipStream_t stream);
int want_latency_path(rgbdfe_ctx* ctx, rgbdfe_ctx::Lane& lane, int32_t n, hipStream_t stream, bool* use, int* chunk_out, PhasePlan* plan);
bool hamming_on_mfma(const rgbdfe_ctx* ctx);
HammingGeometry hamming_geometry(const rgbdfe_ctx* ctx, uint32_t n, uint32_t max_nq, uint32_t max_nt);
uint32_t launch_hamming(rgbdfe_ctx* ctx, const PairWork* d_work, uint32_t* d_keys, uint32_t n, HammingGeometry geom, hipStream_t stream);
// ... 323 lines not shown
```

rgbdslam_v2_amd/csrc/rgbdfe_internal.h:

```cpp
#pragma once
#include <hip/hip_runtime.h>
#include <stdint.h>

#include "rgbdfe.h"

namespace rgbdfe {

struct PairWork {
  uint32_t q_slot, t_slot;
  uint32_t nq, nt;
  uint32_t uid;
  int32_t qid, tid;
  uint32_t pad;
};
static_assert(sizeof(PairWork) == 32, "PairWork layout");

constexpr uint32_t kNoMatchKey = (257u << 16) | 0xFFFFu;

struct RansacConst {
  int32_t max_matches, min_matches, ransac_iterations;
  float max_dist_m;
  double sq_max_dist;
  double depth_cov;
  double raster_cov_x;
  double raster_cov_y;
  uint32_t seed;
  int32_t g2o_iterations;
};

struct HammingGeometry { uint32_t qblocks, tsplit, wide, shape; };
HammingGeometry hamming_nn_geometry(uint32_t n_pairs, uint32_t max_nq, uint32_t max_nt, uint32_t key_planes_capacity);
uint32_t launch_hamming_nn(const uint32_t* desc_pool, const PairWork* work, uint32_t* keys,
                           uint32_t max_kp, uint32_t n_pairs, HammingGeometry geom, hipStream_t stream);
uint32_t hamming_mfma_tiles_per_slot(uint32_t max_kp);
size_t hamming_mfma_slab_bytes(uint32_t max_nodes, uint32_t max_kp);
void launch_hamming_expand(const uint32_t* node_rows, uint32_t* slab, uint32_t slot, uint32_t max_kp, uint32_t n,
                           hipStream_t stream);
HammingGeometry hamming_mfma_geometry(uint32_t n_pairs, uint32_t max_nq, uint32_t max_nt, uint32_t key_planes_capacity,
                                      int pipe_wide, int wide_shape);
uint32_t launch_hamming_mfma(const uint32_t* slab, const PairWork* work, uint32_t* keys, uint32_t max_kp,
                             uint32_t n_pairs, HammingGeometry geom, int mode, hipStream_t stream);
void launch_place_votes(const uint32_t* keys, uint32_t planes, uint32_t max_kp, const PairWork* work, const uint32_t* seg,
                        uint32_t n_queries, uint32_t max_nq, uint32_t k_neighbours, uint32_t max_hd, uint32_t* votes,
                        hipStream_t stream);
void launch_select_ransac(const float4* xyz_pool, const PairWork* work, const uint32_t* keys,
                          uint32_t key_planes, rgbdfe_match_result* results, uint32_t max_kp,
                          uint32_t n_pairs, const RansacConst& rc, struct PairPrep* prep, double* ec_pool,
                          hipStream_t stream);
struct IterRec {
  float rR[9], rt[3];
  uint64_t rmask[5];
  double rerr;
  int32_t rn;
  int32_t pad;
};
struct IterSum {
  double rerr;
  int32_t rn;
  int32_t pad;
};
struct alignas(16) PairPrep {
  float M[RGBDFE_MAX_MATCHES * 7];
  uint64_t w_nonzero[RGBDFE_MASK_WORDS];
  int32_t n_all;
  float pmax;
  uint32_t fast_alpha;
  uint32_t pad;
};
struct WalkState {
  int32_t state;
  int32_t it, real_iterations, valid_iterations;
  int32_t best_idx;
  int32_t best_n;
  float rmse;
  int32_t speculate;
};
struct RecordPlan {
  IterRec* recs = nullptr;
  IterSum* sums = nullptr;
  WalkState* walk = nullptr;
  const PairPrep* prep = nullptr;
  double* ec_pool = nullptr;
  const uint64_t* vmask = nullptr;
  int vmask_words = 0;
};
size_t select_ransac_ec_region_bytes();
struct SplitPlan {
  IterRec* recs = nullptr;
  IterSum* sums = nullptr;
  uint64_t* vmask = nullptr;
  WalkState* walk = nullptr;
  const PairPrep* prep = nullptr;
  int vmask_words = 0;
  int phased = 0;
  int n_phases = 1;
  int phase_ends[4] = {0, 0, 0, 0};
  int n_shares = 1;
  int share_iters = 0;
  uint8_t* preclass = nullptr;
  int preclass_iters = 0;
  uint32_t* unit_counter = nullptr;
  uint32_t* order_cnt = nullptr;
  uint32_t* order = nullptr;
};
constexpr int kOrderBuckets = 64;
__host__ __device__ inline int order_bucket(int n) { return n < 32 ? n : (32 + (n - 32) / 8 < kOrderBuckets ? 32 + (n - 32) / 8 : kOrderBuckets - 1); }
void launch_ransac_hyp(const PairWork* work, uint32_t n_pairs, const RansacConst& rc, const SplitPlan& plan, hipStream_t stream);
void launch_ransac_refine(uint32_t n_pairs, const RansacConst& rc, const SplitPlan& plan, hipStream_t stream);
int ransac_split_words_per_pair(int ransac_iterations);
int ransac_split_max_share();
int ransac_split_wgs();
int ransac_split_init();
inline size_t ransac_split_mask_bytes(size_t rec_capacity, size_t max_pairs) { return (rec_capacity / 64 + (5 + 32) * max_pairs + 64 + 64) * 8; }
inline uint32_t* ransac_split_order_cnt(IterRec* recs, size_t n_pairs, int ransac_iterations) {
  const size_t I = ransac_iterations > 0 ? (size_t)ransac_iterations : 0, n_recs = n_pairs * I;
  uint64_t* vmask = reinterpret_cast<uint64_t*>(reinterpret_cast<IterSum*>(recs + n_recs) + n_recs);
  uint8_t* preclass = reinterpret_cast<uint8_t*>(vmask + n_pairs * (size_t)ransac_split_words_per_pair(ransac_iterations));
  return reinterpret_cast<uint32_t*>(preclass + ((n_pairs + 8 + 7) & ~(size_t)7));
}
void launch_compact_edges(const rgbdfe_match_result* in, uint32_t n, rgbdfe_match_result* out, int32_t* out_index,
                          int32_t index_scale, int32_t index_offset, int32_t* d_dst, int32_t* d_count, hipStream_t stream);
void launch_compact_pack(const rgbdfe_match_result* in, uint32_t n, rgbdfe_compact_result* out, hipStream_t stream);
void launch_pack_inliers(const rgbdfe_match_result* in, uint32_t n, uint32_t n_headers, void* stream_out, int32_t* d_total,
                         hipStream_t stream);
void launch_g2o_refine(const PairWork* work, rgbdfe_match_result* results, uint32_t n_pairs, const RansacConst& rc,
                       const struct PairPrep* prep, const float* kp_pool, uint32_t max_kp, double* ec_pool, hipStream_t stream);
void launch_select_ransac_latency(const float4* xyz_pool, const PairWork* work, const uint32_t* keys,
                                  uint32_t key_planes, rgbdfe_match_result* results, uint32_t max_kp,
                                  uint32_t n_pairs, const RansacConst& rc, PairPrep* prep, IterRec* recs, WalkState* walk,
                                  double* ec_pool, int chunk_iters, const int* phase_ends, int n_phases, hipStream_t stream);
void launch_select_ransac_sift_latency(const float4* xyz_pool, const PairWork* work, uint16_t* sm_q,
                                       uint16_t* sm_t, float* sm_d, const int32_t* sm_n, float* all_dist,
                                       rgbdfe_match_result* results, uint32_t max_kp, uint32_t n_pairs,
                                       const RansacConst& rc, PairPrep* prep, IterRec* recs, WalkState* walk,
                                       double* ec_pool, int chunk_iters, const int* phase_ends, int n_phases, hipStream_t stream);
void launch_select_ransac_sift(const float4* xyz_pool, const PairWork* work, uint16_t* sm_q,
                               uint16_t* sm_t, float* sm_d, const int32_t* sm_n,
                               float* all_dist, rgbdfe_match_result* results, uint32_t max_kp,
                               uint32_t n_pairs, const RansacConst& rc, struct PairPrep* prep, double* ec_pool,
                               hipStream_t stream);
void launch_sift_dot(const uint16_t* bf16_pool, const PairWork* work, uint32_t max_kp,
                     uint32_t n_pairs, uint32_t max_nq, uint32_t max_nt, uint32_t key_kinds,
                     uint32_t* row_part, uint32_t* col_part, uint2* col_blocks, hipStream_t stream);
void launch_sift_finish(const float* f32_pool, const PairWork* work, uint32_t max_kp,
                        uint32_t n_pairs, const uint32_t* row_part, uint32_t* col_part, const uint2* col_blocks,
                        uint16_t* sm_q, uint16_t* sm_t, float* sm_d, int32_t* sm_n,
                        hipStream_t stream);
size_t sift_col_block_bytes_per_pair();
void launch_l2_knn2(const float* f32_pool, const PairWork* work, uint32_t max_kp, uint32_t n_pairs, uint32_t max_nq,
                    uint32_t* knn, hipStream_t stream);
void launch_l2_ratio(const PairWork* work, uint32_t max_kp, uint32_t n_pairs, const uint32_t* knn, uint32_t* claim,
                     double max_ratio, uint16_t* sm_q, uint16_t* sm_t, float* sm_d, int32_t* sm_n, hipStream_t stream);
void launch_sift_quantise(const float* f32, uint16_t* bf16, size_t n_elems, hipStream_t stream);
void launch_project_to_3d(const float* kp_xy, int n_kp, const float* depth, int rows, int cols,
                          float fxinv, float fyinv, float cx, float cy, double depth_scaling,
                          int max_keypoints, int32_t* kept_idx, float4* xyz1, int32_t* n_out,
                          hipStream_t stream, bool truncate = false, const float* z_gathered = nullptr);
constexpr int kProjectFramesMax = 32;
struct ProjectFrames { int n_frames; int off[kProjectFramesMax]; int n[kProjectFramesMax]; };
void launch_project_to_3d_frames(const ProjectFrames& fr, const float* kpxy, int rows, int cols, float fxinv, float fyinv,
                                 float cx, float cy, double depth_scaling, int max_keypoints, int32_t* kept_idx, float4* xyz1,
                                 int32_t* n_out, hipStream_t stream);
void launch_min_depth(const float* kp_xys, int n_kp, const float* depth, int rows, int cols, float* z_out,
                      hipStream_t stream);
void launch_project_cloud(const float* kp_xy, int n_kp, const float4* pts, bool gathered, int rows, int cols,
                          double maximum_depth, int max_keypoints, int32_t* kept_idx, float4* xyz1, int32_t* n_out,
                          hipStream_t stream);
struct EmmJob {
  const float4* new_samples;
  const float* old_z;
  float T[12];
  float fx, fy, cx, cy;
};
void launch_depth_to_mono8_f32(const float* depth, size_t n, uint8_t* mono8, hipStream_t stream);
void launch_depth_u16(const uint16_t* depth_mm, size_t n, uint8_t* mono8, float* depth_m, hipStream_t stream);
void launch_create_cloud(const float* depth, int rows, int cols, const uint8_t* rgb, int channels,
                         int encoding_bgr, float fxinv, float fyinv, float cx, float cy, double depth_scaling,
                         float min_depth, int s, int ch, int cw, float4* cloud, float* zplane, hipStream_t stream);
void launch_decimate_cloud(const float4* cloud, int ch, int cw, int skip_step, float4* out, hipStream_t stream);
void launch_emm(const EmmJob* jobs, int n_jobs, int ch, int cw, int skip_step, double d_lo, double d_hi,
                uint32_t* counts, hipStream_t stream);
constexpr uint32_t kMapTile = 1024;
struct MapNode {
  const float4* cloud;
  int64_t first_point;
  uint32_t n_points;
  uint32_t first_tile;
  float R[9], t[3];
};
static_assert(sizeof(MapNode) == 72, "MapNode layout");
void launch_map_raster(const MapNode* nodes, const uint32_t* tile_node, uint32_t n_tiles, bool clip, float md2, float4* out,
                       hipStream_t stream);
void launch_map_count_scan(const MapNode* nodes, const uint32_t* tile_node, uint32_t n_nodes, uint32_t n_tiles, bool clip,
                           float md2, uint32_t* tile_count, int64_t* tile_first, int64_t* node_first, hipStream_t stream);
void launch_map_write(const MapNode* nodes, const uint32_t* tile_node, uint32_t n_tiles, const int64_t* tile_first, bool clip,
                      float md2, float4* out, hipStream_t stream);
constexpr uint32_t kVoxTile = 1024;
constexpr uint32_t kVoxSortTile = 4096;
struct VoxHeader {
  float min_p[3], max_p[3];
  uint32_t n_valid, n_cells;
};
struct VoxGrid {
  float inv;
  float min_b[3];
  uint32_t mul1, mul2;
  uint32_t flip;
};
void launch_vox_stats(const float4* pts, uint32_t n, float* tile_box, uint32_t* tile_count, uint32_t* tile_first, VoxHeader* hdr,
                      hipStream_t stream);
void launch_vox_keys(const float4* pts, uint32_t n, const VoxGrid& g, const uint32_t* tile_first, uint32_t* keys, uint32_t* idx,
                     hipStream_t stream);
int launch_vox_sort(uint32_t n, int passes, uint32_t* keys[2], uint32_t* idx[2], uint32_t* hist, uint32_t* digit_total,
                    hipStream_t stream);
void launch_vox_heads(const uint32_t* keys, uint32_t n, uint32_t* tile_count, uint32_t* tile_first, uint32_t* cell_start,
                      VoxHeader* hdr, hipStream_t stream);
void launch_vox_centroids(const float4* pts, const uint32_t* idx, const uint32_t* cell_start, uint32_t n_cells, float4* out,
                          float* zplane, hipStream_t stream);
constexpr uint64_t kOctoEmptyKey = ~0ull;
constexpr uint32_t kOctoNoLeaf = 0xffffffffu;
constexpr uint32_t kOctoMaxSteps = 3u * 65536u;
struct OctoTable {
  unsigned long long* key;
  float* value;
  uint32_t* colour;
  uint32_t* mark;
  uint32_t cap;
};
struct OctoCtl {
  uint32_t overflow;
  uint32_t n_done;
  uint32_t n_leaves;
  uint32_t pad;
};
struct OctoCloud {
  float R[9], t[3];
  double inv_res, res;
  double max_range;
  float hit, miss, clamp_min, clamp_max;
  uint32_t epoch;
};
struct OctoScratch {
  uint32_t* keys[2];
  uint32_t* idx[2];
  uint32_t *hist, *digits, *tile_count, *tile_first, *cell_start;
  VoxHeader* hdr;
};
void launch_octo_cloud(const OctoTable& tb, OctoCtl* ctl, const float4* pts, uint32_t n, const OctoCloud& c, int sort_passes,
                       const OctoScratch& s, hipStream_t stream);
void launch_octo_rehash(const OctoTable& from, const OctoTable& to, OctoCtl* ctl, hipStream_t stream);
struct OctoLeafIn {
  unsigned long long key;
  float value;
  uint32_t colour;
};
void launch_octo_set_leaves(const OctoLeafIn* src, uint32_t n, const OctoTable& to, OctoCtl* ctl, uint32_t* dup, hipStream_t stream);
constexpr uint32_t kTreeTile = 1024;
struct TreeHdr {
  uint32_t cnt[17];
  uint32_t n_nodes;
  uint32_t n_out;
  uint32_t dup;
  uint32_t pad[4];
};
struct TreeLevel {
  float* value;
  uint32_t* colour;
  uint32_t* first;
};
struct TreeScratch {
  TreeHdr* hdr;
  unsigned long long *code, *scode;
  uint32_t* slot;
  uint32_t* keys[2];
  uint32_t* idx[2];
  uint32_t *hist, *digits, *tile_count, *tile_first;
  uint32_t *top, *off;
  TreeLevel level[2];
};
// ... 28 lines not shown
```

rgbdslam_v2_amd/csrc/select_ransac.hip:

```cpp
#include "ransac_device.h"

namespace rgbdfe {

#ifdef RGBDFE_LDS_ONLY_SYNC
__device__ __forceinline__ void wave_sync() {
  __builtin_amdgcn_wave_barrier();
  asm volatile("s_waitcnt lgkmcnt(0)" ::: "memory");
  __builtin_amdgcn_wave_barrier();
}
__device__ __forceinline__ void wave_sync_global() {
  __builtin_amdgcn_wave_barrier();
  asm volatile("s_waitcnt vmcnt(0) lgkmcnt(0)" ::: "memory");
  __builtin_amdgcn_wave_barrier();
}
#else
__device__ __forceinline__ void wave_sync() { __syncthreads(); }
__device__ __forceinline__ void wave_sync_global() { __syncthreads(); }
#endif


struct SelBuf {
  uint32_t mqt[RGBDFE_MAX_MATCHES];
  uint32_t mhd[RGBDFE_MAX_MATCHES];
  uint32_t cnt[128];
};
struct ScoreBuf {
  uint16_t cand[RGBDFE_MAX_MATCHES];
  uint32_t mbits[2 * kRounds];
};
constexpr int kStageBlk = 32;
constexpr int kStageRow = kStageBlk + 2;
struct SumStage {
  double v[kSlots][kStageRow];
};
union Scratch {
  ScoreBuf sc;
  FitBuf fit;
  SumStage sum;
};
struct Hyp {
  float R[9], t[3];
  uint64_t mask[kRounds];
  int n;
  int nan;
  double err;
};
struct Slot {
  float R[9], t[3];
  float rR[9], rt[3];
  uint64_t rmask[kRounds];
  uint64_t cmask[kRounds];
  double rerr;
  int rn;
  int cn;
  int active;
  int round;
  int iter;
  int pad;
};
struct __attribute__((aligned(16))) RansacLds {
  Scratch u;
  alignas(16) float M[RGBDFE_MAX_MATCHES * kRec];
  Slot slot[kSlots];
  Hyp best;
};



#ifdef RGBDFE_PROFILE_PHASES
#define PH_DECL uint64_t ph_t0 = __builtin_readcyclecounter(); uint64_t ph[22] = {0, 0, 0, 0, 0, 0, 0, 0, 0, 0, 0, 0, 0, 0, 0, 0, 0, 0, 0, 0, 0, 0};
#define PH_MARK(i) { uint64_t ph_t1 = __builtin_readcyclecounter(); ph[i] += ph_t1 - ph_t0; ph_t0 = ph_t1; }
#define PH_COUNT(i) { ph[i] += 1; }
#define PH_ADDX(i, v) { ph[i] += (uint64_t)(v); }
#define PH_ARG , uint64_t* ph, uint64_t& ph_t0
#define PH_PASS , ph, ph_t0
#else
#define PH_DECL
#define PH_MARK(i)
#define PH_COUNT(i)
#define PH_ADDX(i, v)
#define PH_ARG
#define PH_PASS
#endif
#define PH_ADD(i, v) PH_ADDX(i, v)


constexpr int kEcRow = RGBDFE_MAX_MATCHES;
constexpr int kEcRegion = kSlots * kEcRow;

__device__ __forceinline__ void score_passes(const float* R, const float* tr, int n_all, uint32_t need,
                                             const RansacConst& rc, RansacLds& lds, float pmax,
                                             double* __restrict__ ec_row, uint64_t* mask, int& n_inl PH_ARG) {
  const int lane = threadIdx.x;
  double Rd[9], td[3];
#pragma unroll
  for (int i = 0; i < 9; ++i) Rd[i] = (double)R[i];
#pragma unroll
  for (int i = 0; i < 3; ++i) td[i] = (double)tr[i];
  const double rcx = rc.raster_cov_x, rcy = rc.raster_cov_y, dc = rc.depth_cov;
  const double smax = rcx > dc ? rcx : dc;
  const double shortcut = 2.0 * (smax + smax);
  ScoreBuf& sb = lds.u.sc;
  float lo_f, hi_f;
  {
    const float u4 = 4.0f * 5.9604645e-8f;
    float es = 0.0f;
#pragma unroll
    for (int i = 0; i < 3; ++i)
      es += u4 * (((fabsf(R[3 * i]) + fabsf(R[3 * i + 1])) + fabsf(R[3 * i + 2]) + 1.0f) * pmax + fabsf(tr[i]));
    const float S = (float)shortcut;
    const float E = 2.0f * ((2.0f * sqrtf(S) * 1.001f) * es + es * es + u4 * S) + 1e-30f;
    lo_f = S * 0.999999f - E;
    hi_f = S * 1.000001f + E;
  }
  int n_cand = 0;
#pragma unroll
  for (int r = 0; r < kRounds; ++r) {
    const int m = r * kWave + lane;
    const float pxf = lds.M[m * kRec + 0], pyf = lds.M[m * kRec + 1], pzf = lds.M[m * kRec + 2];
    const float qxf = lds.M[m * kRec + 3], qyf = lds.M[m * kRec + 4], qzf = lds.M[m * kRec + 5];
    const bool pre = (m < n_all) && !(pzf == 0.0f || qzf == 0.0f) && !(__builtin_isnan(pzf) || __builtin_isnan(qzf));
    const float f0 = __builtin_fmaf(R[0], pxf, __builtin_fmaf(R[1], pyf, __builtin_fmaf(R[2], pzf, tr[0]))) - qxf;
    const float f1 = __builtin_fmaf(R[3], pxf, __builtin_fmaf(R[4], pyf, __builtin_fmaf(R[5], pzf, tr[1]))) - qyf;
    const float f2 = __builtin_fmaf(R[6], pxf, __builtin_fmaf(R[7], pyf, __builtin_fmaf(R[8], pzf, tr[2]))) - qzf;
    const float dsq_f = __builtin_fmaf(f0, f0, __builtin_fmaf(f1, f1, f2 * f2));
    const bool sure_in = dsq_f < lo_f, sure_out = dsq_f > hi_f;
    bool cand = pre && sure_in;
    if (__ballot(pre && !(sure_in || sure_out)) != 0ull) {
      const double a0 = (double)pxf, a1 = (double)pyf, a2 = (double)pzf;
      const double d0 = (((Rd[0] * a0 + Rd[1] * a1) + Rd[2] * a2) + td[0]) - (double)qxf;
      const double d1 = (((Rd[3] * a0 + Rd[4] * a1) + Rd[5] * a2) + td[1]) - (double)qyf;
      const double d2 = (((Rd[6] * a0 + Rd[7] * a1) + Rd[8] * a2) + td[2]) - (double)qzf;
      const double dsq = (d0 * d0 + d1 * d1) + d2 * d2;
      cand = pre && !(dsq > shortcut) && !__builtin_isnan(d2);
    }
    const uint64_t cm = __ballot(cand);
    if (cand) sb.cand[n_cand + (int)lane_rank(cm)] = (uint16_t)m;
    n_cand += __popcll(cm);
  }
  if (lane < 2 * kRounds) sb.mbits[lane] = 0u;
  wave_sync();
  n_inl = 0;
#pragma unroll
  for (int r = 0; r < kRounds; ++r) mask[r] = 0ull;
  PH_ADD(13, n_cand)
  if ((uint32_t)n_cand < need) { PH_COUNT(15) return; }
  for (int k0 = 0; k0 < n_cand; k0 += kWave) {
    const int k = k0 + lane;
    const bool act = k < n_cand;
    const int m = act ? (int)sb.cand[k] : 0;
    const double a0 = (double)lds.M[m * kRec + 0], a1 = (double)lds.M[m * kRec + 1], a2 = (double)lds.M[m * kRec + 2];
    const double b0 = (double)lds.M[m * kRec + 3], b1 = (double)lds.M[m * kRec + 4], b2 = (double)lds.M[m * kRec + 5];
    double d[3];
    d[0] = (((Rd[0] * a0 + Rd[1] * a1) + Rd[2] * a2) + td[0]) - b0;
    d[1] = (((Rd[3] * a0 + Rd[4] * a1) + Rd[5] * a2) + td[1]) - b1;
    d[2] = (((Rd[6] * a0 + Rd[7] * a1) + Rd[8] * a2) + td[2]) - b2;
    double e = DBL_MAX;
    {
      const double c1[3] = {rcx * a2, rcy * a2, dc};
      const double c2[3] = {rcx * b2, rcy * b2, dc};
      double A[9];
#pragma unroll
      for (int i = 0; i < 3; ++i)
#pragma unroll
        for (int kk = 0; kk < 3; ++kk) A[i * 3 + kk] = Rd[kk * 3 + i] * c1[kk];
      const double S00 = ((A[0] * Rd[0] + A[1] * Rd[3]) + A[2] * Rd[6]) + c2[0];
      const double S10 = (A[3] * Rd[0] + A[4] * Rd[3]) + A[5] * Rd[6];
      const double S11 = ((A[3] * Rd[1] + A[4] * Rd[4]) + A[5] * Rd[7]) + c2[1];
      const double S20 = (A[6] * Rd[0] + A[7] * Rd[3]) + A[8] * Rd[6];
      const double S21 = (A[6] * Rd[1] + A[7] * Rd[4]) + A[8] * Rd[7];
      const double S22 = ((A[6] * Rd[2] + A[7] * Rd[5]) + A[8] * Rd[8]) + c2[2];
      bool ok, unsafe;
      double ee = mahal_llt_fast(S00, S10, S11, S20, S21, S22, d, ok, unsafe);
      if (__ballot(act && unsafe) != 0ull)
        ee = mahal_llt_ieee(S00, S10, S11, S20, S21, S22, d, ok);
      if (ok && (ee >= 0.0)) e = ee;
    }
    const bool inl = act && !(e > rc.sq_max_dist) && (e >= 0.0);
    const uint64_t im = __ballot(inl);
    if (inl) {
      ec_row[n_inl + (int)lane_rank(im)] = e;
      atomicOr(&sb.mbits[m >> 5], 1u << (m & 31));
    }
    n_inl += __popcll(im);
  }
  wave_sync();
#pragma unroll
  for (int r = 0; r < kRounds; ++r) {
    const uint32_t lo = __builtin_amdgcn_readfirstlane(sb.mbits[2 * r]);
    const uint32_t hi = __builtin_amdgcn_readfirstlane(sb.mbits[2 * r + 1]);
    mask[r] = ((uint64_t)hi << 32) | lo;
  }
  PH_ADD(14, n_inl)
  wave_sync();
}

__device__ __forceinline__ double sum_rows(const double* __restrict__ ec_region, RansacLds& lds, int lane, int n_mine,
                                           int n_max PH_ARG) {
  SumStage& st = lds.u.sum;
  const int col = lane & (kStageBlk - 1);
  int row[4], n_row[4];
#pragma unroll
  for (int j = 0; j < 4; ++j) {
    row[j] = (j * kWave + lane) / kStageBlk;
    n_row[j] = __shfl(n_mine, min(row[j], kSlots - 1));
    if (row[j] >= kSlots) n_row[j] = -1;
  }
  const int nb = (n_max + kStageBlk - 1) / kStageBlk;
  auto fetch = [&](double* g, int b) {
    const int idx = max(min(b, nb - 1), 0) * kStageBlk + col;
#pragma unroll
    for (int j = 0; j < 4; ++j) {
      g[j] = 0.0;
      uint32_t off = (uint32_t)(((j * kWave + lane) / kStageBlk) * kEcRow + idx);
      asm volatile("" : "+v"(off));
      if (idx < n_row[j]) g[j] = ec_region[off];
    }
  };
  const double* mine = st.v[min(lane, kSlots - 1)];
  double sum = 0.0;
  auto block = [&](double* g, int b) {
    const int idx = b * kStageBlk + col;
#pragma unroll
    for (int j = 0; j < 4; ++j)
      if (n_row[j] >= 0) st.v[row[j]][col] = idx < n_row[j] ? g[j] : 0.0;
    wave_sync();
    asm volatile("" ::: "memory");
    fetch(g, b + 2);
    asm volatile("" ::: "memory");
#pragma unroll
    for (int i = 0; i < kStageBlk; i += 2) {
      const double2 v = *reinterpret_cast<const double2*>(mine + i);
      sum += v.x;
      sum += v.y;
    }
    asm volatile("" : "+v"(sum) :: "memory");
    wave_sync();
  };
  double g0[4], g1[4];
  PH_MARK(20)
  wave_sync_global();
  PH_MARK(21)
  fetch(g0, 0);
  fetch(g1, 1);
#ifdef RGBDFE_PROFILE_PHASES
  asm volatile("s_waitcnt vmcnt(0)" ::: "memory");
  PH_MARK(0)
#endif
  for (int b = 0; b < nb; b += 2) {
    block(g0, b);
    if (b + 1 < nb) block(g1, b + 1);
  }
  return sum;
}


__device__ __forceinline__ void score_hypothesis(const float* R, const float* tr, int n_all, uint32_t need,
                                                 const RansacConst& rc, RansacLds& lds, float pmax,
                                                 double* __restrict__ ec_region, uint64_t* mask, int& n_inl,
                                                 double& err PH_ARG) {
  score_passes(R, tr, n_all, need, rc, lds, pmax, ec_region, mask, n_inl PH_PASS);
  err = 1e9;
  if ((uint32_t)n_inl < need || n_inl < 3) return;
  const double sum = uniform_f64(sum_rows(ec_region, lds, threadIdx.x, threadIdx.x == 0 ? n_inl : 0, n_inl PH_PASS));
  err = sqrt(sum / (double)n_inl);
}



__device__ __forceinline__ void hyp_store(Hyp& h, const float* R, const float* t, const uint64_t* mask,
                                          int n, int nan, double err) {
  if (threadIdx.x == 0) {
#pragma unroll
    for (int i = 0; i < 9; ++i) h.R[i] = R[i];
#pragma unroll
    for (int i = 0; i < 3; ++i) h.t[i] = t[i];
#pragma unroll
    for (int r = 0; r < kRounds; ++r) h.mask[r] = mask[r];
    h.n = n;
    h.nan = nan;
    h.err = err;
  }
}


struct SiftMatchList {
  const uint16_t* q;
  const uint16_t* t;
  const float* d;
  const int32_t* n;
  float* all_dist;
};

constexpr int kSortThreads = 256;
__global__ __launch_bounds__(kSortThreads) void sift_sort_kernel(uint16_t* __restrict__ sm_q, uint16_t* __restrict__ sm_t,
                                                                 float* __restrict__ sm_d, const int32_t* __restrict__ sm_n,
                                                                 uint32_t max_kp, uint32_t n_pairs, int max_matches) {
  constexpr int kTile = 2048;
  __shared__ uint64_t s_key[kTile];
  __shared__ uint32_t s_qt[RGBDFE_MAX_MATCHES], s_d[RGBDFE_MAX_MATCHES];
  const uint32_t pair = blockIdx.x;
  if (pair >= n_pairs) return;
  const int tid = threadIdx.x;
  uint16_t* __restrict__ sq = sm_q + (size_t)pair * max_kp;
  uint16_t* __restrict__ st = sm_t + (size_t)pair * max_kp;
  float* __restrict__ sd = sm_d + (size_t)pair * max_kp;
  const int n = sm_n[pair];
  const int n_all = min(n, max_matches);
  if (n <= kTile) {
    int n_pad = 2;
    while (n_pad < n) n_pad <<= 1;
    for (int j = tid; j < n_pad; j += kSortThreads)
      s_key[j] = j < n ? (((uint64_t)__float_as_uint(sd[j]) << 32) | ((uint64_t)sq[j] << 16) | (uint64_t)st[j]) : ~0ull;
    __syncthreads();
    for (int k = 2; k <= n_pad; k <<= 1)
      for (int j = k >> 1; j > 0; j >>= 1) {
        for (int i = tid; i < (n_pad >> 1); i += kSortThreads) {
          const int lo = ((i & ~(j - 1)) << 1) | (i & (j - 1)), hi = lo | j;
          const uint64_t a = s_key[lo], b = s_key[hi];
          const bool up = (lo & k) == 0;
          if ((a > b) == up) {
            s_key[lo] = b;
            s_key[hi] = a;
          }
        }
        __syncthreads();
      }
    for (int m = tid; m < n_all; m += kSortThreads) {
      const uint64_t key = s_key[m];
      sq[m] = (uint16_t)((key >> 16) & 0xFFFFu);
      st[m] = (uint16_t)(key & 0xFFFFu);
      sd[m] = __uint_as_float((uint32_t)(key >> 32));
    }
    return;
  }
  auto key_of = [&](int i) { return ((uint64_t)__float_as_uint(sd[i]) << 16) | (uint64_t)sq[i]; };
  for (int base = 0; base < n; base += kSortThreads) {
    const int i = base + tid;
    const bool act = i < n;
    const uint64_t ki = act ? key_of(i) : 0ull;
    int rank = 0;
    for (int t0 = 0; t0 < n; t0 += kTile) {
      const int tn = min(kTile, n - t0);
      __syncthreads();
      for (int j = tid; j < tn; j += kSortThreads) s_key[j] = key_of(t0 + j);
      __syncthreads();
      int j = 0;
      for (; j + 8 <= tn; j += 8) {
#pragma unroll
        for (int u = 0; u < 8; ++u) rank += s_key[j + u] < ki ? 1 : 0;
      }
      for (; j < tn; ++j) rank += s_key[j] < ki ? 1 : 0;
    }
    if (act && rank < max_matches) {
      s_qt[rank] = (uint32_t)sq[i] | ((uint32_t)st[i] << 16);
      s_d[rank] = __float_as_uint(sd[i]);
    }
  }
  __syncthreads();
  for (int m = tid; m < n_all; m += kSortThreads) {
    sq[m] = (uint16_t)(s_qt[m] & 0xFFFFu);
    st[m] = (uint16_t)(s_qt[m] >> 16);
    sd[m] = __uint_as_float(s_d[m]);
  }
}

constexpr int kWhole = 0, kReplay = 1;

template <bool SIFT>
__global__ __launch_bounds__(kWave) void pair_prep_kernel(
    const float4* __restrict__ xyz_pool, const PairWork* __restrict__ work,
    const uint32_t* __restrict__ keys, uint32_t key_planes, const SiftMatchList sm,
    rgbdfe_match_result* __restrict__ results, uint32_t max_kp, uint32_t n_pairs,
    const RansacConst rc, PairPrep* __restrict__ prep, uint32_t* __restrict__ zero64) {
  __shared__ SelBuf sel;
  const uint32_t pair = blockIdx.x;
  if (pair >= n_pairs) return;
  const int lane = threadIdx.x;
  if (pair == 0 && zero64 != nullptr) zero64[lane] = 0u;
  const PairWork w = work[pair];
  rgbdfe_match_result* __restrict__ out = results + pair;
  PairPrep* __restrict__ pp = prep + pair;
  const int max_matches = rc.max_matches;
  int n_all;

  if (!SIFT) {
  const uint32_t nq = w.nq;
  const uint32_t* __restrict__ kin = keys + (size_t)pair * key_planes * max_kp;
  auto load_key = [&](uint32_t i) {
    uint32_t k = kin[i];
    for (uint32_t pl = 1; pl < key_planes; ++pl) k = min(k, kin[(size_t)pl * max_kp + i]);
    return k;
  };
  sel.cnt[lane] = 0;
  sel.cnt[lane + 64] = 0;
  wave_sync();
  for (uint32_t base = 0; base < nq; base += kWave) {
    const uint32_t i = base + lane;
    if (i < nq) {
      const uint32_t hd = load_key(i) >> 16;
      if (hd < 128u) atomicAdd(&sel.cnt[hd], 1u);
    }
  }
  wave_sync();
  uint32_t total;
  uint32_t cut_hd;
  {
    const uint32_t a = sel.cnt[2 * lane], b = sel.cnt[2 * lane + 1];
    uint32_t incl = a + b;
#pragma unroll
    for (int off = 1; off < kWave; off <<= 1) {
      uint32_t v = __shfl_up(incl, off);
      if (lane >= off) incl += v;
    }
    const uint32_t excl = incl - (a + b);
    total = __builtin_amdgcn_readlane(incl, 63);
    const uint32_t s0 = excl, s1 = excl + a;
    uint32_t c = 128u;
    if (s1 >= (uint32_t)max_matches) c = 2 * lane + 1;
    if (s0 >= (uint32_t)max_matches) c = 2 * lane;
#pragma unroll
    for (int off = 32; off >= 1; off >>= 1) c = min(c, (uint32_t)__shfl_xor(c, off));
    cut_hd = c;
    wave_sync();
    sel.cnt[2 * lane] = s0;
    sel.cnt[2 * lane + 1] = s1;
  }
  wave_sync();
  n_all = (int)min(total, (uint32_t)max_matches);
  for (uint32_t base = 0; base < nq; base += kWave) {
    const uint32_t i = base + lane;
    uint32_t key = i < nq ? load_key(i) : 0xFFFFFFFFu;
    const uint32_t hd = key >> 16;
    const bool valid = hd < cut_hd;
    uint64_t same = __ballot(valid);
    if (same == 0ull) continue;
#pragma unroll
    for (int b = 0; b < 7; ++b) {
      const bool bit = (hd >> b) & 1u;
      const uint64_t bal = __ballot(bit);
      same &= bit ? bal : ~bal;
    }
    const uint32_t rank = lane_rank(same);
    const uint32_t cnt_same = __popcll(same);
    uint32_t pos = 0;
    if (valid) pos = sel.cnt[hd] + rank;
    wave_sync();
    if (valid && rank == 0) sel.cnt[hd] = pos + cnt_same;
    if (valid && pos < (uint32_t)max_matches) {
      sel.mqt[pos] = i | ((key & 0xFFFFu) << 16);
      sel.mhd[pos] = hd;
    }
    wave_sync();
  }
  wave_sync();
  } else {
    const uint16_t* __restrict__ sq = sm.q + (size_t)pair * max_kp;
    const uint16_t* __restrict__ st = sm.t + (size_t)pair * max_kp;
    const float* __restrict__ sd = sm.d + (size_t)pair * max_kp;
    n_all = min(sm.n[pair], max_matches);
#pragma unroll
    for (int r = 0; r < kRounds; ++r) {
      const int m = r * kWave + lane;
      if (m < n_all) {
        sel.mqt[m] = (uint32_t)sq[m] | ((uint32_t)st[m] << 16);
        sel.mhd[m] = __float_as_uint(sd[m]);
      }
    }
    wave_sync();
  }

  const float4* __restrict__ qxyz = xyz_pool + (size_t)w.q_slot * max_kp;
  const float4* __restrict__ txyz = xyz_pool + (size_t)w.t_slot * max_kp;
  bool w_plain = false;
  float pmax = 0.0f;
#pragma unroll
  for (int r = 0; r < kRounds; ++r) {
    const int m = r * kWave + lane;
    float4 p = make_float4(0.f, 0.f, 0.f, 1.f), q = make_float4(0.f, 0.f, 0.f, 1.f);
    uint32_t qt = 0, hd = 0;
    if (m < n_all) {
      qt = sel.mqt[m];
      hd = sel.mhd[m];
      p = qxyz[qt & 0xFFFFu];
      q = txyz[qt >> 16];
    }
    pmax = fmaxf(pmax, fmaxf(fmaxf(fmaxf(fabsf(p.x), fabsf(p.y)), fabsf(p.z)),
                             fmaxf(fmaxf(fabsf(q.x), fabsf(q.y)), fabsf(q.z))));
    float* __restrict__ rec = pp->M + m * kRec;
    rec[0] = p.x; rec[1] = p.y; rec[2] = p.z;
    rec[3] = q.x; rec[4] = q.y; rec[5] = q.z;
    const float wgt = 1.0f / (p.z * q.z);
    rec[6] = wgt;
    {
      const uint32_t ex = (__float_as_uint(wgt) >> 23) & 0xFFu;
      w_plain |= (m < n_all) && (wgt != 0.0f) && (ex < 127u - 40u || ex > 127u + 40u);
      const uint64_t nz = __ballot(wgt != 0.0f);
      if (lane == 0) pp->w_nonzero[r] = nz;
    }
    out->all_q[m] = (uint16_t)(qt & 0xFFFFu);
    out->all_t[m] = (uint16_t)(qt >> 16);
    if (SIFT) {
      out->all_hd[m] = 0;
      sm.all_dist[(size_t)pair * RGBDFE_MAX_MATCHES + m] = __uint_as_float(hd);
    } else {
      out->all_hd[m] = (uint8_t)hd;
    }
  }
  const bool fast_alpha = (__ballot(w_plain) == 0ull);
#pragma unroll
  for (int d = 32; d >= 1; d >>= 1) pmax = fmaxf(pmax, __shfl_xor(pmax, d));
  if (lane == 0) {
    pp->n_all = n_all;
    pp->pmax = pmax;
    pp->fast_alpha = fast_alpha ? 1u : 0u;
    pp->pad = 0u;
  }
}

#ifdef RGBDFE_PADNOPS
__global__ void rgbdfe_pad_kernel(int* p) {
#pragma unroll
  for (int i = 0; i < RGBDFE_PADNOPS; ++i) asm volatile("s_nop 0");
  if (p) *p = 1;
}
#endif



template <int MODE>
__global__ __launch_bounds__(kWave) __attribute__((amdgpu_waves_per_eu(3, 3))) void select_ransac_kernel(
    const PairWork* __restrict__ work, rgbdfe_match_result* __restrict__ results, uint32_t n_pairs,
    const RansacConst rc, const RecordPlan plan) {
  __shared__ RansacLds lds;
  const uint32_t pair = blockIdx.x;
  if (pair >= n_pairs) return;
  IterRec* __restrict__ rec_pair = MODE == kWhole ? nullptr : plan.recs + (size_t)pair * (size_t)rc.ransac_iterations;
  IterSum* __restrict__ sum_pair = MODE == kWhole ? nullptr : plan.sums + (size_t)pair * (size_t)rc.ransac_iterations;
  const int lane = threadIdx.x;
  const PairWork w = work[pair];
  rgbdfe_match_result* __restrict__ out = results + pair;
  double* __restrict__ ec_region = plan.ec_pool + (size_t)pair * kEcRegion;
  PH_DECL

  const PairPrep* __restrict__ pp = plan.prep + pair;
  const int n_all = pp->n_all;
  const float pmax = pp->pmax;
  const bool fast_alpha = pp->fast_alpha != 0u;
  uint64_t w_nonzero[kRounds];
#pragma unroll
  for (int r = 0; r < kRounds; ++r) w_nonzero[r] = pp->w_nonzero[r];
  auto load_points = [&]() {
    const float4* __restrict__ src = reinterpret_cast<const float4*>(pp->M);
    float4* __restrict__ dst = reinterpret_cast<float4*>(lds.M);
    constexpr int kVec = RGBDFE_MAX_MATCHES * kRec / 4;
#pragma unroll
    for (int i = 0; i < (kVec + kWave - 1) / kWave; ++i) {
      const int v = i * kWave + lane;
      if (v < kVec) dst[v] = src[v];
    }
    wave_sync();
  };
  if (MODE != kReplay) load_points();

  PH_MARK(1)
  const float IR[9] = {1, 0, 0, 0, 1, 0, 0, 0, 1}, It[3] = {0, 0, 0};
  const uint64_t zero_mask[kRounds] = {0, 0, 0, 0, 0};
  hyp_store(lds.best, IR, It, zero_mask, 0, 0, 0.0);
  int best_n = 0;
  float rmse = 0.0f;
  int valid_iterations = 0, real_iterations = 0;
  bool found = false;

  if (n_all > rc.min_matches) {
    uint32_t thr = (uint32_t)rc.min_matches;
    if ((double)thr > 0.75 * (double)n_all) thr = (uint32_t)(0.75 * (double)n_all);
    auto max_dist_d = [&]() { float f = rc.max_dist_m; asm volatile("" : "+v"(f)); return (double)f; };
    rmse = 1e6f;
    const uint32_t seed_uid = mix32(mix32(rc.seed ^ 0x9E3779B9u) + w.uid * 0x85EBCA6Bu);

    float hypR[9], hypt[3];
    bool hyp_nan = true;
    bool hyp_viable = false;
    uint64_t viable_mask = 0ull;
    int hyp_base = -kWave;
    bool done = false;

    auto gen_hypotheses = [&](int k0) {
        hyp_base = k0;
        const uint32_t iter = (uint32_t)(k0 + lane);
        uint32_t ids[4] = {0, 0, 0, 0};
        int cnt = 0;
        {
          int safety_net = 0;
          uint32_t kk = 0;
          const uint32_t n = (uint32_t)n_all;
          while (cnt < 4) {
            uint32_t id1 = rand31(seed_uid, iter, kk) % n;
            uint32_t id2 = rand31(seed_uid, iter, kk + 1) % n;
            kk += 2;
            if (id1 > id2) id1 = id2;
            const bool dup = (cnt > 0 && ids[0] == id1) || (cnt > 1 && ids[1] == id1) ||
                             (cnt > 2 && ids[2] == id1);
            if (!dup) {
              uint32_t v = id1;
#pragma unroll
              for (int s4 = 0; s4 < 4; ++s4) {
                if (s4 < cnt) {
                  if (ids[s4] > v) { uint32_t tmp = ids[s4]; ids[s4] = v; v = tmp; }
                } else if (s4 == cnt) {
                  ids[s4] = v;
                }
              }
              ++cnt;
            }
            if (++safety_net > 10000) break;
          }
        }
        Tfc acc;
        acc.reset();
#pragma unroll
        for (int s4 = 0; s4 < 4; ++s4)
          if (s4 < cnt) acc.add(lds.M, (int)ids[s4]);
        tfc_get_transformation(acc, hypR, hypt);
        hyp_nan = has_nan12(hypR, hypt);
        hyp_viable = !hyp_nan && prescreen_may_pass(hypR, hypt, lds.M, n_all, pmax, rc) >= thr;
        viable_mask = __ballot(hyp_viable);
        PH_MARK(2)
    };
    auto open_slot = [&](int g, int k) {
      if (hyp_base < 0 || k < hyp_base || k >= hyp_base + kWave) gen_hypotheses(k);
      const int hl = k - hyp_base;
      float R0[9], t0[3];
#pragma unroll
      for (int i = 0; i < 9; ++i) R0[i] = bcast_f(hypR[i], hl);
#pragma unroll
      for (int i = 0; i < 3; ++i) t0[i] = bcast_f(hypt[i], hl);
      const bool nan0 = ((viable_mask >> hl) & 1ull) == 0ull;
      if (lane == 0) {
        Slot& sl = lds.slot[g];
#pragma unroll
        for (int i = 0; i < 9; ++i) { sl.R[i] = R0[i]; sl.rR[i] = IR[i]; }
#pragma unroll
        for (int i = 0; i < 3; ++i) { sl.t[i] = t0[i]; sl.rt[i] = 0.f; }
#pragma unroll
        for (int r = 0; r < kRounds; ++r) sl.rmask[r] = 0ull;
        sl.rerr = 1e6;
        sl.rn = 0;
        sl.active = nan0 ? 0 : 1;
        sl.round = 0;
        sl.iter = k;
      }
    };
    auto refine_round = [&]() -> bool {
        int cn_mine = 0;
        int n_sum_max = 0;
        for (int g = 0; g < kSlots; ++g) {
          Slot& sl = lds.slot[g];
          if (__builtin_amdgcn_readfirstlane(sl.active) == 0) continue;
          float curR[9], curt[3];
#pragma unroll
          for (int i = 0; i < 9; ++i) curR[i] = sl.R[i];
#pragma unroll
          for (int i = 0; i < 3; ++i) curt[i] = sl.t[i];
          uint64_t inl_mask[kRounds];
          int n_inl;
          PH_MARK(5)
          const uint32_t need = max(thr, (uint32_t)__builtin_amdgcn_readfirstlane(sl.rn));
          score_passes(curR, curt, n_all, need, rc, lds, pmax, ec_region + g * kEcRow, inl_mask, n_inl PH_PASS);
          PH_MARK(3)
          PH_COUNT(6)
          if (lane == 0) {
#pragma unroll
            for (int r = 0; r < kRounds; ++r) sl.cmask[r] = inl_mask[r];
            sl.cn = n_inl;
          }
          if (!((uint32_t)n_inl < need || n_inl < 3)) {
            if (lane == g) cn_mine = n_inl;
            n_sum_max = max(n_sum_max, n_inl);
          }
        }
        wave_sync();
        PH_MARK(5)
        PH_COUNT(18)
        PH_ADDX(19, n_sum_max)
#ifdef RGBDFE_FENCE_SUMS
        __builtin_amdgcn_fence(__ATOMIC_ACQUIRE, "agent");
#endif
        const double sum_mine = n_sum_max > 0 ? sum_rows(ec_region, lds, lane, cn_mine, n_sum_max PH_PASS) : 0.0;
        const double err_mine = cn_mine > 0 ? sqrt(sum_mine / (double)cn_mine) : 1e9;
        PH_MARK(11)
        bool still = false;
// ... 99 lines not shown
        const IterRec& r = rec_pair[wr.best_idx];
        Hyp& b = lds.best;
#pragma unroll
        for (int i = 0; i < 9; ++i) b.R[i] = r.rR[i];
#pragma unroll
        for (int i = 0; i < 3; ++i) b.t[i] = r.rt[i];
#pragma unroll
        for (int q = 0; q < kRounds; ++q) b.mask[q] = r.rmask[q];
        b.n = r.rn;
        b.nan = 0;
        b.err = r.rerr;
      }
      wave_sync();
    } else {
    for (; !done && it < rc.ransac_iterations && n_all >= 4;) {
      const int k0 = real_iterations;
      const int G = (k0 == 0) ? 1 : kSlots;
      for (int g = 0; g < G; ++g) open_slot(g, k0 + g);
      wave_sync();
      while (refine_round()) {}
      for (int g = 0; g < G; ++g) {
        if (!(it < rc.ransac_iterations)) { done = true; break; }
        real_iterations++;
        const Slot& sl = lds.slot[g];
        const int refined_n = __builtin_amdgcn_readfirstlane(sl.rn);
        const double refined_error = sl.rerr;
        if (refined_n > 0) {
          valid_iterations++;
          if (refined_error <= (double)rmse && refined_n >= best_n && (uint32_t)refined_n >= thr) {
            rmse = (float)refined_error;
            wave_sync();
            if (lane == 0) {
              Hyp& b = lds.best;
#pragma unroll
              for (int i = 0; i < 9; ++i) b.R[i] = sl.rR[i];
#pragma unroll
              for (int i = 0; i < 3; ++i) b.t[i] = sl.rt[i];
#pragma unroll
              for (int r = 0; r < kRounds; ++r) b.mask[r] = sl.rmask[r];
              b.n = refined_n;
              b.nan = 0;
              b.err = refined_error;
            }
            wave_sync();
            best_n = refined_n;
            int n_all_here = n_all;
            asm volatile("" : "+v"(n_all_here));
            const double n_all_d = (double)n_all_here;
            if ((double)refined_n > n_all_d * 0.5) it += 10;
            if ((double)refined_n > n_all_d * 0.75) it += 10;
            if ((double)refined_n > n_all_d * 0.8) { done = true; break; }
          }
        }
        ++it;
      }
    }
    }
    if (valid_iterations == 0) {
      if (MODE == kReplay) load_points();
      uint64_t inl_mask[kRounds];
      int n_inl;
      double inlier_error;
      score_hypothesis(IR, It, n_all, thr + 1u, rc, lds, pmax, ec_region, inl_mask, n_inl, inlier_error PH_PASS);
      if ((uint32_t)n_inl > thr && inlier_error < max_dist_d()) {
        hyp_store(lds.best, IR, It, inl_mask, n_inl, 0, inlier_error);
        best_n = n_inl;
        rmse = (float)inlier_error;
        valid_iterations++;
      }
    }
    found = (uint32_t)best_n >= thr;
  }
  wave_sync();

  if (lane == 0) {
    const Hyp& b = lds.best;
    out->n_all = n_all;
    out->n_inl = best_n;
    out->rmse = rmse;
#pragma unroll
    for (int i = 0; i < 3; ++i) {
#pragma unroll
      for (int j = 0; j < 3; ++j) out->trafo[j * 4 + i] = b.R[i * 3 + j];
      out->trafo[12 + i] = b.t[i];
      out->trafo[i * 4 + 3] = 0.0f;
    }
    out->trafo[15] = 1.0f;
    out->pad0 = 0;
#ifdef RGBDFE_DEBUG_CLASS
    if (MODE == kReplay) out->pad0 = (uint32_t)plan.walk[pair].speculate;
#endif
    out->valid_iterations = valid_iterations;
    out->real_iterations = real_iterations;
    if (found) {
      out->id1 = w.tid;
      out->id2 = w.qid;
      out->info_scale = (double)((float)best_n / (rmse * rmse));
    } else {
      out->id1 = -1;
      out->id2 = -1;
      out->info_scale = 0.0;
    }
#pragma unroll
    for (int r = 0; r < kRounds; ++r) out->inlier_mask[r] = b.mask[r];
#ifdef RGBDFE_PROFILE_PHASES
    PH_MARK(5)
    uint64_t* dbg = reinterpret_cast<uint64_t*>(out->all_q);
    for (int i = 0; i < 16; ++i) dbg[i] = ph[i];
#endif
  }
}

void launch_select_ransac(const float4* xyz_pool, const PairWork* work, const uint32_t* keys,
                          uint32_t key_planes, rgbdfe_match_result* results, uint32_t max_kp,
                          uint32_t n_pairs, const RansacConst& rc, PairPrep* prep, double* ec_pool, hipStream_t stream) {
  if (n_pairs == 0) return;
  SiftMatchList none{};
  hipLaunchKernelGGL(pair_prep_kernel<false>, dim3(n_pairs), dim3(kWave), 0, stream, xyz_pool, work, keys, key_planes,
                     none, results, max_kp, n_pairs, rc, prep, (uint32_t*)nullptr);
  RecordPlan plan{};
  plan.prep = prep;
  plan.ec_pool = ec_pool;
  hipLaunchKernelGGL(select_ransac_kernel<kWhole>, dim3(n_pairs), dim3(kWave), 0, stream, work, results, n_pairs, rc,
                     plan);
}

static void launch_sift_prep(const float4* xyz_pool, const PairWork* work, uint16_t* sm_q, uint16_t* sm_t, float* sm_d,
                             const int32_t* sm_n, float* all_dist, rgbdfe_match_result* results, uint32_t max_kp,
                             uint32_t n_pairs, const RansacConst& rc, PairPrep* prep, uint32_t* zero64, hipStream_t stream) {
  hipLaunchKernelGGL(sift_sort_kernel, dim3(n_pairs), dim3(kSortThreads), 0, stream, sm_q, sm_t, sm_d, sm_n, max_kp, n_pairs,
                     rc.max_matches);
  SiftMatchList sm{sm_q, sm_t, sm_d, sm_n, all_dist};
  hipLaunchKernelGGL(pair_prep_kernel<true>, dim3(n_pairs), dim3(kWave), 0, stream, xyz_pool, work,
                     (const uint32_t*)nullptr, 1u, sm, results, max_kp, n_pairs, rc, prep, zero64);
}

void launch_select_ransac_sift(const float4* xyz_pool, const PairWork* work, uint16_t* sm_q,
                               uint16_t* sm_t, float* sm_d, const int32_t* sm_n,
                               float* all_dist, rgbdfe_match_result* results, uint32_t max_kp,
                               uint32_t n_pairs, const RansacConst& rc, PairPrep* prep, double* ec_pool,
                               hipStream_t stream) {
  if (n_pairs == 0) return;
  launch_sift_prep(xyz_pool, work, sm_q, sm_t, sm_d, sm_n, all_dist, results, max_kp, n_pairs, rc, prep, nullptr, stream);
  RecordPlan plan{};
  plan.prep = prep;
  plan.ec_pool = ec_pool;
  hipLaunchKernelGGL(select_ransac_kernel<kWhole>, dim3(n_pairs), dim3(kWave), 0, stream, work, results, n_pairs, rc,
                     plan);
}

static void launch_record_replay(const PairWork* work, rgbdfe_match_result* results, uint32_t n_pairs,
                                 const RansacConst& rc, const PairPrep* prep, IterRec* recs, WalkState* walk,
                                 double* ec_pool, int chunk_iters, const int* phase_ends, int n_phases,
                                 hipStream_t stream) {
  const int I = rc.ransac_iterations;
  const size_t n_recs = (size_t)n_pairs * (size_t)(I > 0 ? I : 0);
  SplitPlan sp{};
  sp.recs = recs; sp.walk = walk; sp.prep = prep;
  sp.sums = reinterpret_cast<IterSum*>(recs + n_recs);
  sp.vmask = reinterpret_cast<uint64_t*>(sp.sums + n_recs);
  sp.vmask_words = ransac_split_words_per_pair(I);
  sp.preclass = reinterpret_cast<uint8_t*>(sp.vmask + (size_t)n_pairs * (size_t)sp.vmask_words);
  sp.order_cnt = ransac_split_order_cnt(recs, n_pairs, I);
  sp.order = sp.order_cnt + kOrderBuckets;
  static const bool no_pre = getenv("RGBDFE_NO_PRECLASS") && atoi(getenv("RGBDFE_NO_PRECLASS")) != 0;
  sp.preclass_iters = (n_phases > 1 && !no_pre) ? phase_ends[0] : 0;
  sp.phased = n_phases > 1 ? 1 : 0;
  sp.n_phases = n_phases < 4 ? n_phases : 4;
  for (int p = 0; p < 4; ++p) sp.phase_ends[p] = p < sp.n_phases ? (p == sp.n_phases - 1 ? I : phase_ends[p]) : I;
  int share = chunk_iters >= 28 ? (I > 0 ? I : 1) : chunk_iters * 4;
  {
    const int buffers = ransac_split_wgs() * 4;
    const int want = (int)((buffers + (int)n_pairs - 1) / (int)(n_pairs > 0 ? n_pairs : 1));
    const int by_want = I > 0 ? (I + want - 1) / (want > 0 ? want : 1) : 1;
    if (by_want > share) share = by_want;
  }
  if (share > ransac_split_max_share()) share = ransac_split_max_share();
  sp.n_shares = sp.phased ? 1 : (I > 0 ? (I + share - 1) / share : 1);
  sp.share_iters = sp.phased ? I : (I > 0 ? (I + sp.n_shares - 1) / sp.n_shares : share);
  sp.unit_counter = reinterpret_cast<uint32_t*>(&walk[n_pairs].it);
  launch_ransac_hyp(work, n_pairs, rc, sp, stream);
  if (I > 0) launch_ransac_refine(n_pairs, rc, sp, stream);
  RecordPlan plan{};
  plan.recs = recs; plan.sums = sp.sums; plan.walk = walk; plan.prep = prep; plan.ec_pool = ec_pool;
  plan.vmask = sp.vmask;
  plan.vmask_words = sp.vmask_words;
  hipLaunchKernelGGL(select_ransac_kernel<kReplay>, dim3(n_pairs), dim3(kWave), 0, stream, work, results, n_pairs, rc,
                     plan);
}

void launch_select_ransac_latency(const float4* xyz_pool, const PairWork* work, const uint32_t* keys,
                                  uint32_t key_planes, rgbdfe_match_result* results, uint32_t max_kp,
                                  uint32_t n_pairs, const RansacConst& rc, PairPrep* prep, IterRec* recs, WalkState* walk,
                                  double* ec_pool, int chunk_iters, const int* phase_ends, int n_phases,
                                  hipStream_t stream) {
  if (n_pairs == 0) return;
  SiftMatchList none{};
  hipLaunchKernelGGL(pair_prep_kernel<false>, dim3(n_pairs), dim3(kWave), 0, stream, xyz_pool, work, keys, key_planes,
                     none, results, max_kp, n_pairs, rc, prep, ransac_split_order_cnt(recs, n_pairs, rc.ransac_iterations));
  launch_record_replay(work, results, n_pairs, rc, prep, recs, walk, ec_pool, chunk_iters, phase_ends, n_phases, stream);
}

void launch_select_ransac_sift_latency(const float4* xyz_pool, const PairWork* work, uint16_t* sm_q,
                                       uint16_t* sm_t, float* sm_d, const int32_t* sm_n, float* all_dist,
                                       rgbdfe_match_result* results, uint32_t max_kp, uint32_t n_pairs,
                                       const RansacConst& rc, PairPrep* prep, IterRec* recs, WalkState* walk,
                                       double* ec_pool, int chunk_iters, const int* phase_ends, int n_phases,
                                       hipStream_t stream) {
  if (n_pairs == 0) return;
  launch_sift_prep(xyz_pool, work, sm_q, sm_t, sm_d, sm_n, all_dist, results, max_kp, n_pairs, rc, prep,
                   ransac_split_order_cnt(recs, n_pairs, rc.ransac_iterations), stream);
  launch_record_replay(work, results, n_pairs, rc, prep, recs, walk, ec_pool, chunk_iters, phase_ends, n_phases, stream);
}

struct GnShared {
  double X[RGBDFE_MAX_MATCHES][3];
  float2 kq[RGBDFE_MAX_MATCHES];
  float2 kt[RGBDFE_MAX_MATCHES];
  uint16_t sel[RGBDFE_MAX_MATCHES];
};

__device__ __forceinline__ void gn_proj(const double* Y, double* e, double* J) {
  const double fx = 521.0, fy = 521.0, cx = 319.5, cy = 239.5;
  const double iz = 1.0 / Y[2];
  e[0] = fx * (Y[0] * iz) + cx;
  e[1] = fy * (Y[1] * iz) + cy;
  e[2] = Y[2];
  J[0] = fx * iz; J[1] = 0.0;     J[2] = -(fx * (Y[0] * iz)) * iz;
  J[3] = 0.0;     J[4] = fy * iz; J[5] = -(fy * (Y[1] * iz)) * iz;
  J[6] = 0.0;     J[7] = 0.0;     J[8] = 1.0;
}

__device__ __forceinline__ void gn_match_terms(const double* X, const double* R1, const double* t1, const double* m1,
                                               const double* m2, double wz, double* acc, double* Hpp_inv, double* bp,
                                               double* Hcp) {
  double e2[3], J2[9], e1[3], Jp1[9];
  gn_proj(X, e2, J2);
#pragma unroll
  for (int i = 0; i < 3; ++i) e2[i] = e2[i] - m2[i];
  const double dX[3] = {X[0] - t1[0], X[1] - t1[1], X[2] - t1[2]};
  double Y[3];
#pragma unroll
  for (int i = 0; i < 3; ++i) Y[i] = (R1[0 * 3 + i] * dX[0] + R1[1 * 3 + i] * dX[1]) + R1[2 * 3 + i] * dX[2];
  gn_proj(Y, e1, Jp1);
#pragma unroll
  for (int i = 0; i < 3; ++i) e1[i] = e1[i] - m1[i];
  double J1p[9], J1c[18];
#pragma unroll
  for (int r = 0; r < 3; ++r)
#pragma unroll
    for (int c = 0; c < 3; ++c)
      J1p[r * 3 + c] = (Jp1[r * 3 + 0] * R1[c * 3 + 0] + Jp1[r * 3 + 1] * R1[c * 3 + 1]) + Jp1[r * 3 + 2] * R1[c * 3 + 2];
  const double Yx[9] = {0.0, -Y[2], Y[1], Y[2], 0.0, -Y[0], -Y[1], Y[0], 0.0};
#pragma unroll
  for (int r = 0; r < 3; ++r) {
#pragma unroll
    for (int c = 0; c < 3; ++c) J1c[r * 6 + c] = -Jp1[r * 3 + c];
#pragma unroll
    for (int c = 0; c < 3; ++c)
      J1c[r * 6 + 3 + c] = 2.0 * ((Jp1[r * 3 + 0] * Yx[0 * 3 + c] + Jp1[r * 3 + 1] * Yx[1 * 3 + c]) + Jp1[r * 3 + 2] * Yx[2 * 3 + c]);
  }
  const double w[3] = {1.0, 1.0, wz};
  double Hpp[9];
#pragma unroll
  for (int a = 0; a < 3; ++a)
#pragma unroll
    for (int b = 0; b < 3; ++b) {
      double s2 = 0.0, s1 = 0.0;
#pragma unroll
      for (int r = 0; r < 3; ++r) { s2 += (J2[r * 3 + a] * w[r]) * J2[r * 3 + b]; s1 += (J1p[r * 3 + a] * w[r]) * J1p[r * 3 + b]; }
      Hpp[a * 3 + b] = s2 + s1;
    }
#pragma unroll
  for (int a = 0; a < 3; ++a) {
    double s2 = 0.0, s1 = 0.0;
#pragma unroll
    for (int r = 0; r < 3; ++r) { s2 += (J2[r * 3 + a] * w[r]) * e2[r]; s1 += (J1p[r * 3 + a] * w[r]) * e1[r]; }
    bp[a] = s2 + s1;
  }
  double Hcc[36], bc[6];
#pragma unroll
  for (int a = 0; a < 6; ++a) {
#pragma unroll
    for (int b = 0; b < 6; ++b) {
      double sacc = 0.0;
#pragma unroll
      for (int r = 0; r < 3; ++r) sacc += (J1c[r * 6 + a] * w[r]) * J1c[r * 6 + b];
      Hcc[a * 6 + b] = sacc;
    }
#pragma unroll
    for (int b = 0; b < 3; ++b) {
      double sacc = 0.0;
#pragma unroll
      for (int r = 0; r < 3; ++r) sacc += (J1c[r * 6 + a] * w[r]) * J1p[r * 3 + b];
      Hcp[a * 3 + b] = sacc;
    }
    double sacc = 0.0;
#pragma unroll
    for (int r = 0; r < 3; ++r) sacc += (J1c[r * 6 + a] * w[r]) * e1[r];
    bc[a] = sacc;
  }
  {
    const double c00 = Hpp[4] * Hpp[8] - Hpp[5] * Hpp[7], c01 = Hpp[5] * Hpp[6] - Hpp[3] * Hpp[8], c02 = Hpp[3] * Hpp[7] - Hpp[4] * Hpp[6];
    const double det = (Hpp[0] * c00 + Hpp[1] * c01) + Hpp[2] * c02;
    const double id = 1.0 / det;
    Hpp_inv[0] = c00 * id; Hpp_inv[3] = c01 * id; Hpp_inv[6] = c02 * id;
    Hpp_inv[1] = (Hpp[2] * Hpp[7] - Hpp[1] * Hpp[8]) * id;
    Hpp_inv[4] = (Hpp[0] * Hpp[8] - Hpp[2] * Hpp[6]) * id;
    Hpp_inv[7] = (Hpp[1] * Hpp[6] - Hpp[0] * Hpp[7]) * id;
    Hpp_inv[2] = (Hpp[1] * Hpp[5] - Hpp[2] * Hpp[4]) * id;
    Hpp_inv[5] = (Hpp[2] * Hpp[3] - Hpp[0] * Hpp[5]) * id;
    Hpp_inv[8] = (Hpp[0] * Hpp[4] - Hpp[1] * Hpp[3]) * id;
  }
  double W[18];
#pragma unroll
  for (int a = 0; a < 6; ++a)
#pragma unroll
    for (int b = 0; b < 3; ++b)
      W[a * 3 + b] = (Hcp[a * 3 + 0] * Hpp_inv[0 * 3 + b] + Hcp[a * 3 + 1] * Hpp_inv[1 * 3 + b]) + Hcp[a * 3 + 2] * Hpp_inv[2 * 3 + b];
  int k = 0;
#pragma unroll
  for (int a = 0; a < 6; ++a)
#pragma unroll
    for (int b = a; b < 6; ++b)
      acc[k++] += Hcc[a * 6 + b] - ((W[a * 3 + 0] * Hcp[b * 3 + 0] + W[a * 3 + 1] * Hcp[b * 3 + 1]) + W[a * 3 + 2] * Hcp[b * 3 + 2]);
#pragma unroll
  for (int a = 0; a < 6; ++a) acc[21 + a] += bc[a] - ((W[a * 3 + 0] * bp[0] + W[a * 3 + 1] * bp[1]) + W[a * 3 + 2] * bp[2]);
}

__device__ __forceinline__ void gn_rot_via_quaternion(const double* Rin, double* Rout) {
  double q[4];
  const double t = Rin[0] + Rin[4] + Rin[8];
  if (t > 0.0) {
    double tt = sqrt(t + 1.0);
    q[3] = 0.5 * tt;
    tt = 0.5 / tt;
    q[0] = (Rin[7] - Rin[5]) * tt;
    q[1] = (Rin[2] - Rin[6]) * tt;
    q[2] = (Rin[3] - Rin[1]) * tt;
  } else {
    const bool i1 = Rin[4] > Rin[0];
    const bool i2 = Rin[8] > (i1 ? Rin[4] : Rin[0]);
    auto pick = [&](auto I, auto J, auto K) {
      constexpr int i = decltype(I)::value, j = decltype(J)::value, k = decltype(K)::value;
      double tt = sqrt(Rin[i * 3 + i] - Rin[j * 3 + j] - Rin[k * 3 + k] + 1.0);
      q[i] = 0.5 * tt;
      tt = 0.5 / tt;
      q[3] = (Rin[k * 3 + j] - Rin[j * 3 + k]) * tt;
      q[j] = (Rin[j * 3 + i] + Rin[i * 3 + j]) * tt;
      q[k] = (Rin[k * 3 + i] + Rin[i * 3 + k]) * tt;
    };
    using std::integral_constant;
    if (i2) pick(integral_constant<int, 2>(), integral_constant<int, 0>(), integral_constant<int, 1>());
    else if (i1) pick(integral_constant<int, 1>(), integral_constant<int, 2>(), integral_constant<int, 0>());
    else pick(integral_constant<int, 0>(), integral_constant<int, 1>(), integral_constant<int, 2>());
  }
  const double nrm = sqrt(((q[0] * q[0] + q[1] * q[1]) + q[2] * q[2]) + q[3] * q[3]);
  for (int i = 0; i < 4; ++i) q[i] = q[i] / nrm;
  const double tx = 2.0 * q[0], ty = 2.0 * q[1], tz = 2.0 * q[2];
  const double twx = tx * q[3], twy = ty * q[3], twz = tz * q[3];
  const double txx = tx * q[0], txy = ty * q[0], txz = tz * q[0];
  const double tyy = ty * q[1], tyz = tz * q[1], tzz = tz * q[2];
  Rout[0] = 1.0 - (tyy + tzz); Rout[1] = txy - twz;          Rout[2] = txz + twy;
  Rout[3] = txy + twz;          Rout[4] = 1.0 - (txx + tzz); Rout[5] = tyz - twx;
  Rout[6] = txz - twy;          Rout[7] = tyz + twx;          Rout[8] = 1.0 - (txx + tyy);
// ... 255 lines not shown
```

Baseline: 4.151 million frame-pairs/s.

## Fuse pair-prep match selection into RANSAC hypothesis kernel and split prescreen across lanes

Moves the per-pair match selection and record building into a shared device helper so it can run inside the hypothesis kernel behind a compile flag, removing a separate prep launch and its global round-trip. When that fused path is on, the order counters are zeroed from the host with a memset, and graph capture is skipped until they are in place. Independently, the hypothesis kernel now handles a partially filled last wave by spreading each hypothesis's prescreen across several lanes and summing with shuffles, and wholly out-of-range waves skip work. The kernel also gains a fixed waves-per-EU occupancy hint. The fusion is off by default, but the partial-wave split and the occupancy attribute are active.

```diff
diff --git a/rgbdslam_v2_amd/csrc/api_batches.hip b/rgbdslam_v2_amd/csrc/api_batches.hip
--- a/rgbdslam_v2_amd/csrc/api_batches.hip
+++ b/rgbdslam_v2_amd/csrc/api_batches.hip
@@ -122,6 +122,7 @@
     if (lane.d_recs) (void)hipFree(lane.d_recs);
     lane.d_recs = nullptr;
     lane.recs_capacity = 0;
+    lane.order_zero = nullptr;
     if (hipMalloc((void**)&lane.d_recs, need_recs * (sizeof(IterRec) + sizeof(IterSum)) +
                                             ransac_split_mask_bytes(need_recs, (size_t)ctx->cfg.max_pairs_per_batch)) == hipSuccess)
       lane.recs_capacity = need_recs;
@@ -240,7 +241,10 @@
   hipError_t launch_err = hipSuccess;
   if (n > 0) {
     if (!d_out) d_out = lane.d_results;
-    const bool graphable = ctx->use_graphs && !sift && !ctx->profiling && piece >= n && ctx->rc.g2o_iterations == 0;
+    const bool host_counters = !sift && select_ransac_counters_by_host();
+    auto counters_at = [&](int32_t m) { return ransac_split_order_cnt(lane.d_recs, (size_t)m, ctx->rc.ransac_iterations); };
+    const bool zero_first = host_counters && latency && pp.n_phases > 1 && lane.order_zero != counters_at(piece < n ? piece : n);
+    const bool graphable = ctx->use_graphs && !sift && !ctx->profiling && piece >= n && ctx->rc.g2o_iterations == 0 && !zero_first;
     const HammingGeometry geom = sift ? HammingGeometry{0, 1, 0}
                                       : hamming_geometry(ctx, (uint32_t)(piece < n ? piece : n), max_nq, max_nt);
     if (!sift && geom.qblocks > 0) { ctx->hamming_wide_last = (int)geom.wide; ctx->hamming_shape_last = (int)geom.shape; }
@@ -263,6 +267,7 @@
         if (le == hipSuccess) {
           ctx->graph_launches++;
           ctx->graph_miss_run = 0;
+          if (host_counters && latency) lane.order_zero = counters_at(n);
         } else {
           (void)hipGetLastError();
           (void)hipGraphExecDestroy(ge->exec); (void)hipGraphDestroy(ge->graph);
@@ -320,6 +325,14 @@
         if (!sift) {
           const uint32_t planes = launch_hamming(ctx, d_work, lane.d_keys, (uint32_t)m, first ? geom : hamming_geometry(ctx, (uint32_t)m, max_nq, max_nt), ls);
           if (ctx->profiling && first) (void)hipEventRecord(pend.b, ls);
+          if (latency && host_counters) {
+            uint32_t* const at = counters_at(m);
+            if (pp.n_phases > 1 && lane.order_zero != at) {
+              const hipError_t ze = hipMemsetAsync(at, 0, sizeof(uint32_t) * kOrderBuckets, ls);
+              if (ze != hipSuccess && launch_err == hipSuccess) launch_err = ze;
+            }
+            lane.order_zero = at;
+          }
           if (latency)
             launch_select_ransac_latency(ctx->d_xyz, d_work, lane.d_keys, planes, d_res, mk, (uint32_t)m, ctx->rc,
                                          lane.d_prep, lane.d_recs, lane.d_walk, lane.d_ec, chunk, pp.ends, pp.n_phases, ls);
@@ -344,6 +357,7 @@
                                lane.d_sm_q, lane.d_sm_t, lane.d_sm_d, lane.d_sm_n, ls);
           }
           if (ctx->profiling && first) (void)hipEventRecord(pend.c, ls);
+          if (latency) lane.order_zero = nullptr;
           if (latency)
             launch_select_ransac_sift_latency(ctx->d_xyz, d_work, lane.d_sm_q, lane.d_sm_t, lane.d_sm_d, lane.d_sm_n,
                                               d_dist, d_res, mk, (uint32_t)m, ctx->rc,
@@ -380,6 +394,7 @@
       break;
     }
     if (launch_err == hipSuccess) launch_err = hipGetLastError();
+    if (launch_err != hipSuccess) lane.order_zero = nullptr;
     if (ctx->profiling) {
       if (launch_err == hipSuccess) ctx->pending.push_back(pend);
       else {
diff --git a/rgbdslam_v2_amd/csrc/pair_prep_device.h b/rgbdslam_v2_amd/csrc/pair_prep_device.h
--- /dev/null
+++ b/rgbdslam_v2_amd/csrc/pair_prep_device.h
@@ -0,0 +1,171 @@
+#pragma once
+#include "ransac_device.h"
+
+namespace rgbdfe {
+
+struct SelBuf {
+  uint32_t mqt[RGBDFE_MAX_MATCHES];
+  uint32_t mhd[RGBDFE_MAX_MATCHES];
+  uint32_t cnt[128];
+};
+
+struct SiftMatchList {
+  const uint16_t* q;
+  const uint16_t* t;
+  const float* d;
+  const int32_t* n;
+  float* all_dist;
+};
+
+template <bool SIFT, bool TO_LDS, class Sync>
+__device__ __forceinline__ int pair_prep_wave(SelBuf& sel, const float4* __restrict__ xyz_pool, const PairWork& w, uint32_t pair,
+                                              const uint32_t* __restrict__ keys, uint32_t key_planes, const SiftMatchList& sm,
+                                              rgbdfe_match_result* __restrict__ out, uint32_t max_kp, const RansacConst& rc,
+                                              PairPrep* __restrict__ pp, float* __restrict__ M_lds, int lane, float& pmax_out,
+                                              Sync sync) {
+  const int max_matches = rc.max_matches;
+  int n_all;
+
+  if (!SIFT) {
+  const uint32_t nq = w.nq;
+  const uint32_t* __restrict__ kin = keys + (size_t)pair * key_planes * max_kp;
+  auto load_key = [&](uint32_t i) {
+    uint32_t k = kin[i];
+    for (uint32_t pl = 1; pl < key_planes; ++pl) k = min(k, kin[(size_t)pl * max_kp + i]);
+    return k;
+  };
+  sel.cnt[lane] = 0;
+  sel.cnt[lane + 64] = 0;
+  sync();
+  for (uint32_t base = 0; base < nq; base += kWave) {
+    const uint32_t i = base + lane;
+    if (i < nq) {
+      const uint32_t hd = load_key(i) >> 16;
+      if (hd < 128u) atomicAdd(&sel.cnt[hd], 1u);
+    }
+  }
+  sync();
+  uint32_t total;
+  uint32_t cut_hd;
+  {
+    const uint32_t a = sel.cnt[2 * lane], b = sel.cnt[2 * lane + 1];
+    uint32_t incl = a + b;
+#pragma unroll
+    for (int off = 1; off < kWave; off <<= 1) {
+      uint32_t v = __shfl_up(incl, off);
+      if (lane >= off) incl += v;
+    }
+    const uint32_t excl = incl - (a + b);
+    total = __builtin_amdgcn_readlane(incl, 63);
+    const uint32_t s0 = excl, s1 = excl + a;
+    uint32_t c = 128u;
+    if (s1 >= (uint32_t)max_matches) c = 2 * lane + 1;
+    if (s0 >= (uint32_t)max_matches) c = 2 * lane;
+#pragma unroll
+    for (int off = 32; off >= 1; off >>= 1) c = min(c, (uint32_t)__shfl_xor(c, off));
+    cut_hd = c;
+    sync();
+    sel.cnt[2 * lane] = s0;
+    sel.cnt[2 * lane + 1] = s1;
+  }
+  sync();
+  n_all = (int)min(total, (uint32_t)max_matches);
+  for (uint32_t base = 0; base < nq; base += kWave) {
+    const uint32_t i = base + lane;
+    uint32_t key = i < nq ? load_key(i) : 0xFFFFFFFFu;
+    const uint32_t hd = key >> 16;
+    const bool valid = hd < cut_hd;
+    uint64_t same = __ballot(valid);
+    if (same == 0ull) continue;
+#pragma unroll
+    for (int b = 0; b < 7; ++b) {
+      const bool bit = (hd >> b) & 1u;
+      const uint64_t bal = __ballot(bit);
+      same &= bit ? bal : ~bal;
+    }
+    const uint32_t rank = lane_rank(same);
+    const uint32_t cnt_same = __popcll(same);
+    uint32_t pos = 0;
+    if (valid) pos = sel.cnt[hd] + rank;
+    sync();
+    if (valid && rank == 0) sel.cnt[hd] = pos + cnt_same;
+    if (valid && pos < (uint32_t)max_matches) {
+      sel.mqt[pos] = i | ((key & 0xFFFFu) << 16);
+      sel.mhd[pos] = hd;
+    }
+    sync();
+  }
+  sync();
+  } else {
+    const uint16_t* __restrict__ sq = sm.q + (size_t)pair * max_kp;
+    const uint16_t* __restrict__ st = sm.t + (size_t)pair * max_kp;
+    const float* __restrict__ sd = sm.d + (size_t)pair * max_kp;
+    n_all = min(sm.n[pair], max_matches);
+#pragma unroll
+    for (int r = 0; r < kRounds; ++r) {
+      const int m = r * kWave + lane;
+      if (m < n_all) {
+        sel.mqt[m] = (uint32_t)sq[m] | ((uint32_t)st[m] << 16);
+        sel.mhd[m] = __float_as_uint(sd[m]);
+      }
+    }
+    sync();
+  }
+
+  const float4* __restrict__ qxyz = xyz_pool + (size_t)w.q_slot * max_kp;
+  const float4* __restrict__ txyz = xyz_pool + (size_t)w.t_slot * max_kp;
+  bool w_plain = false;
+  float pmax = 0.0f;
+#pragma unroll
+  for (int r = 0; r < kRounds; ++r) {
+    const int m = r * kWave + lane;
+    float4 p = make_float4(0.f, 0.f, 0.f, 1.f), q = make_float4(0.f, 0.f, 0.f, 1.f);
+    uint32_t qt = 0, hd = 0;
+    if (m < n_all) {
+      qt = sel.mqt[m];
+      hd = sel.mhd[m];
+      p = qxyz[qt & 0xFFFFu];
+      q = txyz[qt >> 16];
+    }
+    pmax = fmaxf(pmax, fmaxf(fmaxf(fmaxf(fabsf(p.x), fabsf(p.y)), fabsf(p.z)),
+                             fmaxf(fmaxf(fabsf(q.x), fabsf(q.y)), fabsf(q.z))));
+    float* __restrict__ rec = pp->M + m * kRec;
+    rec[0] = p.x; rec[1] = p.y; rec[2] = p.z;
+    rec[3] = q.x; rec[4] = q.y; rec[5] = q.z;
+    const float wgt = 1.0f / (p.z * q.z);
+    rec[6] = wgt;
+    if (TO_LDS) {
+      float* __restrict__ lrec = M_lds + m * kRec;
+      lrec[0] = p.x; lrec[1] = p.y; lrec[2] = p.z;
+      lrec[3] = q.x; lrec[4] = q.y; lrec[5] = q.z;
+      lrec[6] = wgt;
+    }
+    {
+      const uint32_t ex = (__float_as_uint(wgt) >> 23) & 0xFFu;
+      w_plain |= (m < n_all) && (wgt != 0.0f) && (ex < 127u - 40u || ex > 127u + 40u);
+      const uint64_t nz = __ballot(wgt != 0.0f);
+      if (lane == 0) pp->w_nonzero[r] = nz;
+    }
+    out->all_q[m] = (uint16_t)(qt & 0xFFFFu);
+    out->all_t[m] = (uint16_t)(qt >> 16);
+    if (SIFT) {
+      out->all_hd[m] = 0;
+      sm.all_dist[(size_t)pair * RGBDFE_MAX_MATCHES + m] = __uint_as_float(hd);
+    } else {
+      out->all_hd[m] = (uint8_t)hd;
+    }
+  }
+  const bool fast_alpha = (__ballot(w_plain) == 0ull);
+#pragma unroll
+  for (int d = 32; d >= 1; d >>= 1) pmax = fmaxf(pmax, __shfl_xor(pmax, d));
+  if (lane == 0) {
+    pp->n_all = n_all;
+    pp->pmax = pmax;
+    pp->fast_alpha = fast_alpha ? 1u : 0u;
+    pp->pad = 0u;
+  }
+  pmax_out = pmax;
+  return n_all;
+}
+
+}
diff --git a/rgbdslam_v2_amd/csrc/ransac_device.h b/rgbdslam_v2_amd/csrc/ransac_device.h
--- a/rgbdslam_v2_amd/csrc/ransac_device.h
+++ b/rgbdslam_v2_amd/csrc/ransac_device.h
@@ -312,7 +312,8 @@
   }
 }
 __device__ __forceinline__ uint32_t prescreen_may_pass_s4(const float* hypR, const float* hypt, const float* __restrict__ S4,
-                                                       int n_all, float pmax, const RansacConst& rc) {
+                                                       int n_all, float pmax, const RansacConst& rc, int blk0 = 0,
+                                                       int blk_step = 1) {
   const float u4 = 4.0f * 5.9604645e-8f;
   float es = 0.0f;
 #pragma unroll
@@ -332,7 +333,7 @@
   for (int i = 0; i < 3; ++i) t2[i] = v2f{hypt[i], hypt[i]};
   const v4f* __restrict__ blocks = reinterpret_cast<const v4f*>(S4);
 #pragma unroll 1
-  for (int m0 = 0; m0 < n_all; m0 += 4) {
+  for (int m0 = 4 * blk0; m0 < n_all; m0 += 4 * blk_step) {
     const v4f* __restrict__ b = blocks + (m0 >> 2) * 6;
     const v4f px = b[0], py = b[1], pz = b[2], qx = b[3], qy = b[4], qz = b[5];
 #pragma unroll
diff --git a/rgbdslam_v2_amd/csrc/ransac_split.hip b/rgbdslam_v2_amd/csrc/ransac_split.hip
--- a/rgbdslam_v2_amd/csrc/ransac_split.hip
+++ b/rgbdslam_v2_amd/csrc/ransac_split.hip
@@ -5,6 +5,7 @@
 #include <vector>
 
 #include "ransac_device.h"
+#include "pair_prep_device.h"
 
 namespace rgbdfe {
 
@@ -302,16 +303,22 @@
 
 }
 
-__global__ __launch_bounds__(kHypThreads) void ransac_hyp_kernel(const PairWork* __restrict__ work, uint32_t n_pairs,
-                                                                const RansacConst rc, const SplitPlan plan) {
+template <bool PREBUILT>
+__global__ __launch_bounds__(kHypThreads) __attribute__((amdgpu_waves_per_eu(7, 7))) void ransac_hyp_kernel(const PairWork* __restrict__ work, uint32_t n_pairs,
+                                                                const RansacConst rc, const SplitPlan plan, const HypSelect hs) {
   __shared__ __attribute__((aligned(16))) float M[RGBDFE_MAX_MATCHES * kRec];
   __shared__ __attribute__((aligned(16))) float S4[(RGBDFE_MAX_MATCHES / 4) * kS4Block];
+  static_assert(sizeof(SelBuf) <= sizeof(S4), "the selection's scratch lives in S4: it is done before the transpose");
+  __shared__ int n_viable_sh;
+  __shared__ int n_all_sh;
+  __shared__ float pmax_sh;
   const uint32_t pair = blockIdx.x;
   if (pair >= n_pairs) return;
+  const PairPrep* __restrict__ pp = plan.prep + pair;
+  int n_all = PREBUILT ? pp->n_all : 0;
   if (pair == 0 && threadIdx.x < sizeof(WalkState) / 4) reinterpret_cast<uint32_t*>(plan.walk + n_pairs)[threadIdx.x] = 0u;
-  const PairPrep* __restrict__ pp = plan.prep + pair;
-  const int n_all = pp->n_all;
-  if (threadIdx.x == 0) {
+  const int tid = threadIdx.x, lane = tid & (kWave - 1);
+  if (tid == kHypThreads - 1) {
     WalkState ws;
     ws.state = rc.ransac_iterations;
     ws.it = 0; ws.real_iterations = 0; ws.valid_iterations = 0;
@@ -320,19 +327,31 @@
     ws.speculate = plan.phased ? 0 : rc.ransac_iterations;
     plan.walk[pair] = ws;
   }
-  if (!(n_all > rc.min_matches && n_all >= 4)) return;
-  const int tid = threadIdx.x, lane = tid & (kWave - 1);
-  {
+  float pmax;
+  if (PREBUILT) {
+    if (!(n_all > rc.min_matches && n_all >= 4)) return;
+    pmax = pp->pmax;
     const float4* __restrict__ src = reinterpret_cast<const float4*>(pp->M);
     float4* __restrict__ dst = reinterpret_cast<float4*>(M);
     for (int v = tid; v < kMVec; v += kHypThreads) dst[v] = src[v];
-  }
-  __shared__ int n_viable_sh;
-  if (tid == 0) n_viable_sh = 0;
-  __syncthreads();
+    if (tid == 0) n_viable_sh = 0;
+    __syncthreads();
+  } else {
+    if (tid < kWave) {
+      const PairWork w = work[pair];
+      float pm;
+      const int na = pair_prep_wave<false, true>(*reinterpret_cast<SelBuf*>(S4), hs.xyz_pool, w, pair, hs.keys, hs.key_planes,
+                                                 SiftMatchList{}, hs.results + pair, hs.max_kp, rc, hs.prep + pair, M, lane, pm,
+                                                 [] { lsync(); });
+      if (tid == 0) { n_all_sh = na; pmax_sh = pm; n_viable_sh = 0; }
+    }
+    __syncthreads();
+    n_all = __builtin_amdgcn_readfirstlane(n_all_sh);
+    pmax = __int_as_float(__builtin_amdgcn_readfirstlane(__float_as_int(pmax_sh)));
+    if (!(n_all > rc.min_matches && n_all >= 4)) return;
+  }
   transpose_records(M, S4, tid, kHypThreads);
   __syncthreads();
-  const float pmax = pp->pmax;
   uint32_t thr = (uint32_t)rc.min_matches;
   if ((double)thr > 0.75 * (double)n_all) thr = (uint32_t)(0.75 * (double)n_all);
   const uint32_t seed_uid = mix32(mix32(rc.seed ^ 0x9E3779B9u) + work[pair].uid * 0x85EBCA6Bu);
@@ -343,6 +362,13 @@
   for (int k0 = 0; k0 < I; k0 += kHypThreads) {
     const int k = k0 + tid;
     const bool in_range = k < I;
+#ifndef RGBDFE_HYP_FULL_PARTIAL_WAVE
+    const int r_wave = __builtin_amdgcn_readfirstlane(I - (k - lane));
+    if (r_wave <= 0) {
+      if (lane == 0) vm_pair[k >> 6] = 0ull;
+      continue;
+    }
+#endif
     const uint32_t iter = (uint32_t)k;
     uint32_t ids[4] = {0, 0, 0, 0};
     int cnt = 0;
@@ -378,7 +404,20 @@
       if (s4 < cnt) acc.add(M, (int)ids[s4]);
     float hypR[9], hypt[3];
     tfc_get_transformation(acc, hypR, hypt);
+#ifdef RGBDFE_HYP_FULL_PARTIAL_WAVE
     const uint32_t may_pass = prescreen_may_pass_s4(hypR, hypt, S4, n_all, pmax, rc);
+#else
+    const int sh = r_wave > kWave / 2 ? 6 : (r_wave <= 1 ? 0 : 32 - __builtin_clz((uint32_t)(r_wave - 1)));
+    {
+      const int src = lane & ((1 << sh) - 1);
+#pragma unroll
+      for (int i = 0; i < 9; ++i) hypR[i] = __shfl(hypR[i], src);
+#pragma unroll
+      for (int i = 0; i < 3; ++i) hypt[i] = __shfl(hypt[i], src);
+    }
+    uint32_t may_pass = prescreen_may_pass_s4(hypR, hypt, S4, n_all, pmax, rc, lane >> sh, kWave >> sh);
+    for (int off = 1 << sh; off < kWave; off <<= 1) may_pass += (uint32_t)__shfl_xor((int)may_pass, off);
+#endif
     const bool viable = in_range && !has_nan12(hypR, hypt) && may_pass >= thr;
     const uint64_t vm = __ballot(viable);
     if (lane == 0) vm_pair[k >> 6] = vm;
@@ -1091,9 +1130,12 @@
 }
 
 void launch_ransac_hyp(const PairWork* work, uint32_t n_pairs, const RansacConst& rc, const SplitPlan& plan,
-                       hipStream_t stream) {
+                       const HypSelect& sel, hipStream_t stream) {
   if (n_pairs == 0) return;
-  hipLaunchKernelGGL(ransac_hyp_kernel, dim3(n_pairs), dim3(kHypThreads), 0, stream, work, n_pairs, rc, plan);
+  if (sel.keys != nullptr)
+    hipLaunchKernelGGL(ransac_hyp_kernel<false>, dim3(n_pairs), dim3(kHypThreads), 0, stream, work, n_pairs, rc, plan, sel);
+  else
+    hipLaunchKernelGGL(ransac_hyp_kernel<true>, dim3(n_pairs), dim3(kHypThreads), 0, stream, work, n_pairs, rc, plan, sel);
 }
 
 int ransac_split_init() {
diff --git a/rgbdslam_v2_amd/csrc/rgbdfe_host.h b/rgbdslam_v2_amd/csrc/rgbdfe_host.h
--- a/rgbdslam_v2_amd/csrc/rgbdfe_host.h
+++ b/rgbdslam_v2_amd/csrc/rgbdfe_host.h
@@ -163,6 +163,7 @@
     hipStream_t stream = nullptr;
     IterRec* d_recs = nullptr;
     size_t recs_capacity = 0;
+    uint32_t* order_zero = nullptr;
     WalkState* d_walk = nullptr;
     PairPrep* d_prep = nullptr;
     double* d_ec = nullptr;
diff --git a/rgbdslam_v2_amd/csrc/rgbdfe_internal.h b/rgbdslam_v2_amd/csrc/rgbdfe_internal.h
--- a/rgbdslam_v2_amd/csrc/rgbdfe_internal.h
+++ b/rgbdslam_v2_amd/csrc/rgbdfe_internal.h
@@ -83,6 +83,7 @@
   double* ec_pool = nullptr;
   const uint64_t* vmask = nullptr;
   int vmask_words = 0;
+  uint32_t* order_cnt = nullptr;
 };
 size_t select_ransac_ec_region_bytes();
 struct SplitPlan {
@@ -105,7 +106,16 @@
 };
 constexpr int kOrderBuckets = 64;
 __host__ __device__ inline int order_bucket(int n) { return n < 32 ? n : (32 + (n - 32) / 8 < kOrderBuckets ? 32 + (n - 32) / 8 : kOrderBuckets - 1); }
-void launch_ransac_hyp(const PairWork* work, uint32_t n_pairs, const RansacConst& rc, const SplitPlan& plan, hipStream_t stream);
+struct HypSelect {
+  const float4* xyz_pool = nullptr;
+  const uint32_t* keys = nullptr;
+  uint32_t key_planes = 1;
+  uint32_t max_kp = 0;
+  rgbdfe_match_result* results = nullptr;
+  struct PairPrep* prep = nullptr;
+};
+void launch_ransac_hyp(const PairWork* work, uint32_t n_pairs, const RansacConst& rc, const SplitPlan& plan, const HypSelect& sel,
+                       hipStream_t stream);
 void launch_ransac_refine(uint32_t n_pairs, const RansacConst& rc, const SplitPlan& plan, hipStream_t stream);
 int ransac_split_words_per_pair(int ransac_iterations);
 int ransac_split_max_share();
@@ -125,6 +135,7 @@
                          hipStream_t stream);
 void launch_g2o_refine(const PairWork* work, rgbdfe_match_result* results, uint32_t n_pairs, const RansacConst& rc,
                        const struct PairPrep* prep, const float* kp_pool, uint32_t max_kp, double* ec_pool, hipStream_t stream);
+bool select_ransac_counters_by_host();
 void launch_select_ransac_latency(const float4* xyz_pool, const PairWork* work, const uint32_t* keys,
                                   uint32_t key_planes, rgbdfe_match_result* results, uint32_t max_kp,
                                   uint32_t n_pairs, const RansacConst& rc, PairPrep* prep, IterRec* recs, WalkState* walk,
diff --git a/rgbdslam_v2_amd/csrc/select_ransac.hip b/rgbdslam_v2_amd/csrc/select_ransac.hip
--- a/rgbdslam_v2_amd/csrc/select_ransac.hip
+++ b/rgbdslam_v2_amd/csrc/select_ransac.hip
@@ -1,4 +1,5 @@
 #include "ransac_device.h"
+#include "pair_prep_device.h"
 
 namespace rgbdfe {
 
@@ -19,11 +20,6 @@
 #endif
 
 
-struct SelBuf {
-  uint32_t mqt[RGBDFE_MAX_MATCHES];
-  uint32_t mhd[RGBDFE_MAX_MATCHES];
-  uint32_t cnt[128];
-};
 struct ScoreBuf {
   uint16_t cand[RGBDFE_MAX_MATCHES];
   uint32_t mbits[2 * kRounds];
@@ -284,14 +280,6 @@
 }
 
 
-struct SiftMatchList {
-  const uint16_t* q;
-  const uint16_t* t;
-  const float* d;
-  const int32_t* n;
-  float* all_dist;
-};
-
 constexpr int kSortThreads = 256;
 __global__ __launch_bounds__(kSortThreads) void sift_sort_kernel(uint16_t* __restrict__ sm_q, uint16_t* __restrict__ sm_t,
                                                                  float* __restrict__ sm_d, const int32_t* __restrict__ sm_n,
@@ -379,143 +367,9 @@
   const int lane = threadIdx.x;
   if (pair == 0 && zero64 != nullptr) zero64[lane] = 0u;
   const PairWork w = work[pair];
-  rgbdfe_match_result* __restrict__ out = results + pair;
-  PairPrep* __restrict__ pp = prep + pair;
-  const int max_matches = rc.max_matches;
-  int n_all;
-
-  if (!SIFT) {
-  const uint32_t nq = w.nq;
-  const uint32_t* __restrict__ kin = keys + (size_t)pair * key_planes * max_kp;
-  auto load_key = [&](uint32_t i) {
-    uint32_t k = kin[i];
-    for (uint32_t pl = 1; pl < key_planes; ++pl) k = min(k, kin[(size_t)pl * max_kp + i]);
-    return k;
-  };
-  sel.cnt[lane] = 0;
-  sel.cnt[lane + 64] = 0;
-  wave_sync();
-  for (uint32_t base = 0; base < nq; base += kWave) {
-    const uint32_t i = base + lane;
-    if (i < nq) {
-      const uint32_t hd = load_key(i) >> 16;
-      if (hd < 128u) atomicAdd(&sel.cnt[hd], 1u);
-    }
-  }
-  wave_sync();
-  uint32_t total;
-  uint32_t cut_hd;
-  {
-    const uint32_t a = sel.cnt[2 * lane], b = sel.cnt[2 * lane + 1];
-    uint32_t incl = a + b;
-#pragma unroll
-    for (int off = 1; off < kWave; off <<= 1) {
-      uint32_t v = __shfl_up(incl, off);
-      if (lane >= off) incl += v;
-    }
-    const uint32_t excl = incl - (a + b);
-    total = __builtin_amdgcn_readlane(incl, 63);
-    const uint32_t s0 = excl, s1 = excl + a;
-    uint32_t c = 128u;
-    if (s1 >= (uint32_t)max_matches) c = 2 * lane + 1;
-    if (s0 >= (uint32_t)max_matches) c = 2 * lane;
-#pragma unroll
-    for (int off = 32; off >= 1; off >>= 1) c = min(c, (uint32_t)__shfl_xor(c, off));
-    cut_hd = c;
-    wave_sync();
-    sel.cnt[2 * lane] = s0;
-    sel.cnt[2 * lane + 1] = s1;
-  }
-  wave_sync();
-  n_all = (int)min(total, (uint32_t)max_matches);
-  for (uint32_t base = 0; base < nq; base += kWave) {
-    const uint32_t i = base + lane;
-    uint32_t key = i < nq ? load_key(i) : 0xFFFFFFFFu;
-    const uint32_t hd = key >> 16;
-    const bool valid = hd < cut_hd;
-    uint64_t same = __ballot(valid);
-    if (same == 0ull) continue;
-#pragma unroll
-    for (int b = 0; b < 7; ++b) {
-      const bool bit = (hd >> b) & 1u;
-      const uint64_t bal = __ballot(bit);
-      same &= bit ? bal : ~bal;
-    }
-    const uint32_t rank = lane_rank(same);
-    const uint32_t cnt_same = __popcll(same);
-    uint32_t pos = 0;
-    if (valid) pos = sel.cnt[hd] + rank;
-    wave_sync();
-    if (valid && rank == 0) sel.cnt[hd] = pos + cnt_same;
-    if (valid && pos < (uint32_t)max_matches) {
-      sel.mqt[pos] = i | ((key & 0xFFFFu) << 16);
-      sel.mhd[pos] = hd;
-    }
-    wave_sync();
-  }
-  wave_sync();
-  } else {
-    const uint16_t* __restrict__ sq = sm.q + (size_t)pair * max_kp;
-    const uint16_t* __restrict__ st = sm.t + (size_t)pair * max_kp;
-    const float* __restrict__ sd = sm.d + (size_t)pair * max_kp;
-    n_all = min(sm.n[pair], max_matches);
-#pragma unroll
-    for (int r = 0; r < kRounds; ++r) {
-      const int m = r * kWave + lane;
-      if (m < n_all) {
-        sel.mqt[m] = (uint32_t)sq[m] | ((uint32_t)st[m] << 16);
-        sel.mhd[m] = __float_as_uint(sd[m]);
-      }
-    }
-    wave_sync();
-  }
-
-  const float4* __restrict__ qxyz = xyz_pool + (size_t)w.q_slot * max_kp;
-  const float4* __restrict__ txyz = xyz_pool + (size_t)w.t_slot * max_kp;
-  bool w_plain = false;
-  float pmax = 0.0f;
-#pragma unroll
-  for (int r = 0; r < kRounds; ++r) {
-    const int m = r * kWave + lane;
-    float4 p = make_float4(0.f, 0.f, 0.f, 1.f), q = make_float4(0.f, 0.f, 0.f, 1.f);
-    uint32_t qt = 0, hd = 0;
-    if (m < n_all) {
-      qt = sel.mqt[m];
-      hd = sel.mhd[m];
-      p = qxyz[qt & 0xFFFFu];
-      q = txyz[qt >> 16];
-    }
-    pmax = fmaxf(pmax, fmaxf(fmaxf(fmaxf(fabsf(p.x), fabsf(p.y)), fabsf(p.z)),
-                             fmaxf(fmaxf(fabsf(q.x), fabsf(q.y)), fabsf(q.z))));
-    float* __restrict__ rec = pp->M + m * kRec;
-    rec[0] = p.x; rec[1] = p.y; rec[2] = p.z;
-    rec[3] = q.x; rec[4] = q.y; rec[5] = q.z;
-    const float wgt = 1.0f / (p.z * q.z);
-    rec[6] = wgt;
-    {
-      const uint32_t ex = (__float_as_uint(wgt) >> 23) & 0xFFu;
-      w_plain |= (m < n_all) && (wgt != 0.0f) && (ex < 127u - 40u || ex > 127u + 40u);
-      const uint64_t nz = __ballot(wgt != 0.0f);
-      if (lane == 0) pp->w_nonzero[r] = nz;
-    }
-    out->all_q[m] = (uint16_t)(qt & 0xFFFFu);
-    out->all_t[m] = (uint16_t)(qt >> 16);
-    if (SIFT) {
-      out->all_hd[m] = 0;
-      sm.all_dist[(size_t)pair * RGBDFE_MAX_MATCHES + m] = __uint_as_float(hd);
-    } else {
-      out->all_hd[m] = (uint8_t)hd;
-    }
-  }
-  const bool fast_alpha = (__ballot(w_plain) == 0ull);
-#pragma unroll
-  for (int d = 32; d >= 1; d >>= 1) pmax = fmaxf(pmax, __shfl_xor(pmax, d));
-  if (lane == 0) {
-    pp->n_all = n_all;
-    pp->pmax = pmax;
-    pp->fast_alpha = fast_alpha ? 1u : 0u;
-    pp->pad = 0u;
-  }
+  float pmax;
+  (void)pair_prep_wave<SIFT, false>(sel, xyz_pool, w, pair, keys, key_planes, sm, results + pair, max_kp, rc, prep + pair,
+                                    nullptr, lane, pmax, [] { wave_sync(); });
 }
 
 #ifdef RGBDFE_PADNOPS
@@ -538,6 +392,8 @@
   IterRec* __restrict__ rec_pair = MODE == kWhole ? nullptr : plan.recs + (size_t)pair * (size_t)rc.ransac_iterations;
   IterSum* __restrict__ sum_pair = MODE == kWhole ? nullptr : plan.sums + (size_t)pair * (size_t)rc.ransac_iterations;
   const int lane = threadIdx.x;
+  static_assert(kOrderBuckets == kWave, "one lane per counter");
+  if (MODE == kReplay && pair == 0 && plan.order_cnt != nullptr) plan.order_cnt[lane] = 0u;
   const PairWork w = work[pair];
   rgbdfe_match_result* __restrict__ out = results + pair;
   double* __restrict__ ec_region = plan.ec_pool + (size_t)pair * kEcRegion;
@@ -943,7 +799,7 @@
 static void launch_record_replay(const PairWork* work, rgbdfe_match_result* results, uint32_t n_pairs,
                                  const RansacConst& rc, const PairPrep* prep, IterRec* recs, WalkState* walk,
                                  double* ec_pool, int chunk_iters, const int* phase_ends, int n_phases,
-                                 hipStream_t stream) {
+                                 const HypSelect& hsel, hipStream_t stream) {
   const int I = rc.ransac_iterations;
   const size_t n_recs = (size_t)n_pairs * (size_t)(I > 0 ? I : 0);
   SplitPlan sp{};
@@ -970,12 +826,13 @@
   sp.n_shares = sp.phased ? 1 : (I > 0 ? (I + share - 1) / share : 1);
   sp.share_iters = sp.phased ? I : (I > 0 ? (I + sp.n_shares - 1) / sp.n_shares : share);
   sp.unit_counter = reinterpret_cast<uint32_t*>(&walk[n_pairs].it);
-  launch_ransac_hyp(work, n_pairs, rc, sp, stream);
+  launch_ransac_hyp(work, n_pairs, rc, sp, hsel, stream);
   if (I > 0) launch_ransac_refine(n_pairs, rc, sp, stream);
   RecordPlan plan{};
   plan.recs = recs; plan.sums = sp.sums; plan.walk = walk; plan.prep = prep; plan.ec_pool = ec_pool;
   plan.vmask = sp.vmask;
   plan.vmask_words = sp.vmask_words;
+  plan.order_cnt = sp.order_cnt;
   hipLaunchKernelGGL(select_ransac_kernel<kReplay>, dim3(n_pairs), dim3(kWave), 0, stream, work, results, n_pairs, rc,
                      plan);
 }
@@ -986,10 +843,25 @@
                                   double* ec_pool, int chunk_iters, const int* phase_ends, int n_phases,
                                   hipStream_t stream) {
   if (n_pairs == 0) return;
+#ifndef RGBDFE_HYP_FUSED_PREP
   SiftMatchList none{};
   hipLaunchKernelGGL(pair_prep_kernel<false>, dim3(n_pairs), dim3(kWave), 0, stream, xyz_pool, work, keys, key_planes,
                      none, results, max_kp, n_pairs, rc, prep, ransac_split_order_cnt(recs, n_pairs, rc.ransac_iterations));
-  launch_record_replay(work, results, n_pairs, rc, prep, recs, walk, ec_pool, chunk_iters, phase_ends, n_phases, stream);
+  const HypSelect hsel{};
+#else
+  HypSelect hsel{};
+  hsel.xyz_pool = xyz_pool; hsel.keys = keys; hsel.key_planes = key_planes; hsel.max_kp = max_kp;
+  hsel.results = results; hsel.prep = prep;
+#endif
+  launch_record_replay(work, results, n_pairs, rc, prep, recs, walk, ec_pool, chunk_iters, phase_ends, n_phases, hsel, stream);
+}
+
+bool select_ransac_counters_by_host() {
+#ifdef RGBDFE_HYP_FUSED_PREP
+  return true;
+#else
+  return false;
+#endif
 }
 
 void launch_select_ransac_sift_latency(const float4* xyz_pool, const PairWork* work, uint16_t* sm_q,
@@ -1001,7 +873,7 @@
   if (n_pairs == 0) return;
   launch_sift_prep(xyz_pool, work, sm_q, sm_t, sm_d, sm_n, all_dist, results, max_kp, n_pairs, rc, prep,
                    ransac_split_order_cnt(recs, n_pairs, rc.ransac_iterations), stream);
-  launch_record_replay(work, results, n_pairs, rc, prep, recs, walk, ec_pool, chunk_iters, phase_ends, n_phases, stream);
+  launch_record_replay(work, results, n_pairs, rc, prep, recs, walk, ec_pool, chunk_iters, phase_ends, n_phases, HypSelect{}, stream);
 }
 
 struct GnShared {
```

Measured after the change: 4.187 million frame-pairs/s, median of 6. No clear change (+0.9%).
